# hungdinhxuan/real-time-deepfake-speech-detection

Hardware: AMD Instinct MI355X
Metric: utterances/sec (4 s @ 16 kHz) (higher is better)
Workload: dtype fp16

## Files before the change

### include/afx.h

```cpp
#ifndef AFX_H_
#define AFX_H_

#include <stddef.h>
#include <stdint.h>

#ifdef __cplusplus
extern "C" {
#endif

typedef struct afx_engine* afx_handle;

enum { AFX_ARCH_SSL = 0, AFX_ARCH_XLSR_AASIST = 1, AFX_ARCH_CONFORMER = 2,
       AFX_ARCH_CONFORMER_HEAD = 3  };
enum { AFX_EXTRACTOR_LAYER_NORM = 0,
       AFX_EXTRACTOR_GROUP_NORM = 1   };
enum { AFX_DT_BF16 = 0, AFX_DT_FP16 = 1, AFX_DT_FP32 = 2,
       AFX_DT_FP16X3 = 3  };

typedef struct afx_config {
  int arch;
  int dtype;
  int n_layers;
  int conf_emb;
  int conf_heads;
  int conf_kernel;
  int conf_blocks;
  int pre_emphasis;
  float pre_emphasis_coef;
  int extractor_mode;
} afx_config;

int afx_create(const afx_config* cfg, afx_handle* out);
void afx_destroy(afx_handle h);
const char* afx_last_error(void);
const char* afx_version(void);
const char* afx_build_id(void);
int afx_hip_versions(int* build, int* runtime);

int afx_load_weight(afx_handle h, const char* name, const float* dev_ptr, const int64_t* shape, int ndim,
                    void* stream);
int afx_finalize(afx_handle h, void* stream);

int afx_num_frames(int n_samples);
size_t afx_workspace_bytes(afx_handle h, int B, int L);
int afx_forward(afx_handle h, const float* wave, int B, int L, float* logits, void* ws, size_t ws_bytes,
                void* stream);
int afx_trunk_forward(afx_handle h, const float* wave, int B, int L, void* ws, size_t ws_bytes, void* stream);
int afx_head_from_workspace(afx_handle h, int B, int L, float* logits, void* ws, size_t ws_bytes, void* stream);
int afx_ssl_forward(afx_handle h, const float* wave, int B, int L, float* feats, void* ws, size_t ws_bytes,
                    void* stream);
size_t afx_ragged_workspace_bytes(afx_handle h, int B, int Lmax);
int afx_forward_ragged(afx_handle h, const float* wave, int B, int Lmax, const int* n_samples, float* logits, void* ws,
                       size_t ws_bytes, void* stream);
int afx_ssl_forward_ragged(afx_handle h, const float* wave, int B, int Lmax, const int* n_samples, float* feats,
                           int* n_frames, void* ws, size_t ws_bytes, void* stream);
size_t afx_tail_workspace_bytes(afx_handle h, int B, int T5);
int afx_tail_forward(afx_handle h, const void* conv5_h, int B, int T5, float* logits, void* ws, size_t ws_bytes,
                     void* stream);
int afx_tail_forward_strided(afx_handle h, const void* conv5_h, long batch_stride, int B, int T5, float* logits, void* ws,
                             size_t ws_bytes, void* stream);
size_t afx_tail_windows_workspace_bytes(afx_handle h, int B, int T5);
int afx_tail_forward_windows(afx_handle h, const void* conv5_h, long long total_elems, const long long* offs, int B, int T5,
                             float* logits, void* ws, size_t ws_bytes, void* stream);
typedef struct afx_kv afx_kv;
int afx_kv_create(afx_handle h, int n_streams, afx_kv** out);
void afx_kv_destroy(afx_kv* kv);
size_t afx_kv_state_bytes(const afx_kv* kv);
size_t afx_kv_workspace_bytes(const afx_kv* kv, int n_frames);
int afx_kv_step(afx_kv* kv, const float* feats6, int n_frames, float* logits, void* ws, size_t ws_bytes, void* stream);
int afx_kv_reset(afx_kv* kv, const int* slots, int n_slots, void* stream);
size_t afx_kv_ragged_workspace_bytes(const afx_kv* kv, int n_max);
int afx_kv_step_ragged(afx_kv* kv, const float* feats6, int n_max, const int* n_frames, float* logits, void* ws, size_t ws_bytes,
                       void* stream);
size_t afx_kv_active_workspace_bytes(const afx_kv* kv, int n_active, int n_max);
int afx_kv_step_active(afx_kv* kv, const int* slots, int n_active, const float* feats6, int n_max, const int* n_frames,
                       float* logits, void* ws, size_t ws_bytes, void* stream);
#define AFX_KV_META 8
size_t afx_kv_slot_bytes(const afx_kv* kv);
int afx_kv_export(afx_kv* kv, const int* slots, int n, void* payload, int* meta, void* stream);
int afx_kv_import(afx_kv* kv, const int* slots, int n, const void* payload, const int* meta, void* stream);
int afx_head_forward(afx_handle h, const float* feats, int B, int T, float* logits, void* ws, size_t ws_bytes,
                     void* stream);
size_t afx_head_workspace_bytes(afx_handle h, int B, int T);
int afx_conformer_forward(afx_handle h, const float* tokens, int B, int T, float* logits, float* embedding, void* ws,
                          size_t ws_bytes, void* stream);
int afx_check_finite(afx_handle h, void* stream);
int afx_enable_taps(afx_handle h, int on);
int afx_tap(afx_handle h, const char* name, float* out, size_t cap_elems, size_t* n_out, void* stream);

int afx_profile_begin(afx_handle h);
int afx_profile_end(afx_handle h, int n_classes, double* ms, double* flops, long long* launches);
int afx_profile_num_classes(void);
const char* afx_profile_class_name(int cls);

int afx_engine_set(afx_handle h, const char* key, int value);
int afx_engine_get(afx_handle h, const char* key, int* value);
int afx_gemm_plan(int M, int N, int K, int rpb, int kchunk, int groups, int flags, int objective, int* out);
int afx_conf_chain_waves(int M, int objective);
int afx_debug_set(const char* key, int value);

int afx_k_gemm(int dtype, const void* A, long lda, const void* W, long ldw, int M, int N, int K, const float* bias,
               int act, float alpha, const float* resid, long ldr, float* out_f, long ldo_f, void* out_h, long ldo_h,
               void* stream);
int afx_k_conv_gemm(int dtype, const void* in_h, const void* Wp, int B, int Tin, int Tout, int Cin, int k, int s,
                    int N, const float* bias, float* out_f, void* stream);
int afx_k_conv_ln_act(int dtype, const void* in_h, const void* Wp, int B, int Tin, int Tout, int Cin, int k, int s,
                      const float* bias, const float* gamma, const float* beta, float eps, int act, float* out_f,
                      void* out_h, void* stream);
int afx_k_pack_linear(int dtype, const float* w, int N, int K, int Kpad, void* out_h, void* stream);
int afx_k_pack_conv(int dtype, const float* w, int N, int Cin, int k, void* out_h, void* stream);
int afx_k_conv0(int dtype, const float* wave, int B, int L, const float* w, const float* bias, const float* gamma,
                const float* beta, int pre_emph, float coef, void* out_h, void* stream);
size_t afx_k_conv0_pack_bytes(void);
int afx_k_conv0_pack(const float* w, const float* bias, void* pack, void* stream);
int afx_k_conv0_packed(int dtype, const float* wave, int B, int L, const void* pack, const float* w, const float* bias,
                       const float* gamma, const float* beta, int pre_emph, float coef, void* out_h, void* stream);
int afx_k_pre_emphasis(const float* x, int B, int L, float coef, float* y, void* stream);
int afx_k_tile_crop(const float* x, const long long* offs, const long long* starts, int B, int duration, float* out,
                    void* stream);
int afx_k_resample(const float* x, const long long* in_offs, const long long* out_offs, int B, long long max_out,
                   const float* taps, int L, int M, int T, float* out, void* stream);
int afx_k_resample_stream(const float* x, int A, int n_in, float* hist, const int* slot, const float* taps, int L, int M,
                          int T, float* out, void* stream);
int afx_k_ingest(const void* stage, long long stage_bytes, const int* hdr, int rows, int max_out, int encoding,
                 const float* taps, int L, int M, int T, float* hist, float* ring, int S, int ring_len, void* stream);
typedef struct afx_ingest_format {
  const float* taps;
  int encoding, L, M, T;
} afx_ingest_format;
int afx_k_ingest_mixed(const void* stage, long long stage_bytes, const int* hdr, int rows, const afx_ingest_format* formats,
                       int n_formats, const int* max_out, float* hist, int Hs, float* ring, int S, int ring_len, void* stream);
int afx_k_ingest_pop(const float* ring, int S, int ring_len, const int* table, int A, int hop, float* out, void* stream);
int afx_k_payload_expand(void* stage, long long stage_bytes, const int* hdr, int rows, int max_n, void* stream);
int afx_k_jitter_place(const void* stage, long long stage_bytes, const int* hdr, int rows, int max_n, int encoding,
                       float* jring, int S, int J, void* stream);
int afx_k_jitter_place_mixed(const void* stage, long long stage_bytes, const int* hdr, int rows, int max_n, float* jring, int S,
                             int J, void* stream);
int afx_k_jitter_conceal(float* jring, int S, int J, const int* hdr, int rows, int max_n, const float* fade, int P, int F,
                         int mode, void* stream);
int afx_k_jitter_release(const float* jring, int S, int J, const int* hdr, int rows, int max_out, const float* taps, int L,
                         int M, int T, float* ring, int ring_len, void* stream);
typedef struct afx_jitter_rate {
  const float* taps;
  const float* fade;
  int L, M, T, J, P, F;
} afx_jitter_rate;
int afx_k_jitter_place_rates(const void* stage, long long stage_bytes, const int* hdr, int rows, int max_n,
                             const afx_jitter_rate* rates, int n_rates, float* jring, int S, int Js, void* stream);
int afx_k_jitter_conceal_rates(float* jring, int S, int Js, const int* hdr, int rows, int max_n, const afx_jitter_rate* rates,
                               int n_rates, int mode, void* stream);
int afx_k_jitter_release_rates(const float* jring, int S, int Js, const int* hdr, int rows, const afx_jitter_rate* rates,
                               int n_rates, const int* max_out, float* ring, int ring_len, void* stream);
int afx_k_jitter_noise(float* jring, int S, int J, const int* hdr, int rows, int max_n, unsigned seed, const float* amp,
                       void* stream);
int afx_k_jitter_noise_rates(float* jring, int S, int Js, const int* hdr, int rows, int max_n, const afx_jitter_rate* rates,
                             int n_rates, unsigned seed, const float* amp, void* stream);
typedef struct afx_jitter_lags {
  int Pmin, Pmax, Wc, P0, Hd;
} afx_jitter_lags;
int afx_k_jitter_pitch(const float* jring, int S, int J, const int* hdr, int rows, int Pmin, int Pmax, int Wc, int P0, int* period,
                       void* stream);
int afx_k_jitter_pitch_rates(const float* jring, int S, int Js, const int* hdr, int rows, const afx_jitter_rate* rates,
                             const afx_jitter_lags* lags, int n_rates, int* period, void* stream);
int afx_k_jitter_conceal_period(float* jring, int S, int J, const int* hdr, int rows, int max_n, const float* gain,
                                const int* period, int Pmin, int Pmax, int P0, int Hd, int F, void* stream);
int afx_k_jitter_conceal_period_rates(float* jring, int S, int Js, const int* hdr, int rows, int max_n, const afx_jitter_rate* rates,
                                      const afx_jitter_lags* lags, int n_rates, const int* period, void* stream);
int afx_k_gate(const float* x, int A, int n, const int* hdr, int frame, float e_floor, float ratio, float rise, int hang,
               float* nf, int* h, float* ring, int S, int ring_len, int* kept, unsigned char* mask, void* stream);
int afx_k_gate_la(const float* x, int A, int n, const int* hdr, int frame, float e_floor, float ratio, float rise, int hang,
                  int pre, float* nf, int* h, int* flags, float* line, float* ring, int* src, int S, int ring_len, int* kept,
                  unsigned char* mask, void* stream);
int afx_k_gate_tone(const float* x, int A, int n, const int* hdr, int frame, float e_floor, float ratio, float rise, int hang,
                    const float* coef, int K, float thr, int confirm, int hold, float* nf, int* h, int* tone_state, float* ring,
                    int S, int ring_len, int* kept, int* ntone, unsigned char* mask, float* tsum, void* stream);
int afx_k_turn(const float* staging, int S, int ring_len, const unsigned char* mask, const int* hdr, int A, int F, int frame,
               int min_frames, int max_frames, float* bufs, int* state, int* totals, int* done, void* stream);
int afx_k_turn_collect(const float* bufs, int S, int max_frames, int frame, const int* rows, int R, float* out, void* stream);
int afx_k_turn_close(const int* slots, int A, int S, int min_frames, int max_frames, int* state, int* totals, int* done,
                     void* stream);
int afx_k_turn_scan(const unsigned char* mask, const long long* offs, int A, int min_frames, int max_frames, int close_end,
                    int* table, int cap, int* row_base, int* totals, int* open, void* stream);
int afx_k_turn_clips(const float* x, const long long* xoffs, int A, int frame, int max_frames, const int* table, int r0, int R,
                     float* out, void* stream);
int afx_k_cascade_store(const float* x, int A, int hop, const int* hdr, float* hist, int S, int window, void* stream);
int afx_k_cascade_select(const float* scores, int stride, const int* hdr, int A, int* wait, int* counts, int S,
                         float threshold, int budget, int cooldown, int* sel, void* stream);
int afx_k_cascade_windows(const float* hist, int S, int window, const int* hdr, int A, const int* sel, int budget,
// ... 42 lines not shown
```

### real-time-deepfake-speech-detection_amd/afx/_lib.py

```python
import ctypes as C
import os

_HERE = os.path.dirname(os.path.abspath(__file__))
LIB_PATH = os.environ.get("AFX_LIB") or os.path.join(os.path.dirname(_HERE), "lib", "libafx.so")

ARCH_SSL, ARCH_XLSR_AASIST, ARCH_CONFORMER, ARCH_CONFORMER_HEAD = 0, 1, 2, 3
DT_BF16, DT_FP16, DT_FP32, DT_FP16X3 = 0, 1, 2, 3
ACT_NONE, ACT_GELU, ACT_SWISH, ACT_SELU = 0, 1, 2, 3
KV_META = 8


class AfxError(RuntimeError):
    pass


class Config(C.Structure):
    _fields_ = [("arch", C.c_int), ("dtype", C.c_int), ("n_layers", C.c_int),
                ("conf_emb", C.c_int), ("conf_heads", C.c_int), ("conf_kernel", C.c_int),
                ("conf_blocks", C.c_int), ("pre_emphasis", C.c_int), ("pre_emphasis_coef", C.c_float),
                ("extractor_mode", C.c_int)]


_P, _I, _L, _F, _Z = C.c_void_p, C.c_int, C.c_long, C.c_float, C.c_size_t


class IngestFormat(C.Structure):
    _fields_ = [("taps", C.c_void_p), ("encoding", C.c_int), ("L", C.c_int), ("M", C.c_int), ("T", C.c_int)]


class JitterRate(C.Structure):
    _fields_ = [("taps", C.c_void_p), ("fade", C.c_void_p), ("L", C.c_int), ("M", C.c_int), ("T", C.c_int), ("J", C.c_int),
                ("P", C.c_int), ("F", C.c_int)]


class JitterLags(C.Structure):
    _fields_ = [("Pmin", C.c_int), ("Pmax", C.c_int), ("Wc", C.c_int), ("P0", C.c_int), ("Hd", C.c_int)]


SIGNATURES = {
    "afx_create": (_I, [C.POINTER(Config), C.POINTER(_P)]),
    "afx_destroy": (None, [_P]),
    "afx_last_error": (C.c_char_p, []),
    "afx_version": (C.c_char_p, []),
    "afx_build_id": (C.c_char_p, []),
    "afx_hip_versions": (_I, [C.POINTER(C.c_int), C.POINTER(C.c_int)]),
    "afx_load_weight": (_I, [_P, C.c_char_p, _P, C.POINTER(C.c_int64), _I, _P]),
    "afx_finalize": (_I, [_P, _P]),
    "afx_num_frames": (_I, [_I]),
    "afx_workspace_bytes": (_Z, [_P, _I, _I]),
    "afx_head_workspace_bytes": (_Z, [_P, _I, _I]),
    "afx_forward": (_I, [_P, _P, _I, _I, _P, _P, _Z, _P]),
    "afx_ssl_forward": (_I, [_P, _P, _I, _I, _P, _P, _Z, _P]),
    "afx_trunk_forward": (_I, [_P, _P, _I, _I, _P, _Z, _P]),
    "afx_head_from_workspace": (_I, [_P, _I, _I, _P, _P, _Z, _P]),
    "afx_head_forward": (_I, [_P, _P, _I, _I, _P, _P, _Z, _P]),
    "afx_ragged_workspace_bytes": (_Z, [_P, _I, _I]),
    "afx_forward_ragged": (_I, [_P, _P, _I, _I, C.POINTER(C.c_int), _P, _P, _Z, _P]),
    "afx_ssl_forward_ragged": (_I, [_P, _P, _I, _I, C.POINTER(C.c_int), _P, C.POINTER(C.c_int), _P, _Z, _P]),
    "afx_tail_workspace_bytes": (_Z, [_P, _I, _I]),
    "afx_tail_forward": (_I, [_P, _P, _I, _I, _P, _P, _Z, _P]),
    "afx_tail_forward_strided": (_I, [_P, _P, _L, _I, _I, _P, _P, _Z, _P]),
    "afx_tail_windows_workspace_bytes": (_Z, [_P, _I, _I]),
    "afx_tail_forward_windows": (_I, [_P, _P, C.c_longlong, C.POINTER(C.c_longlong), _I, _I, _P, _P, _Z, _P]),
    "afx_conformer_forward": (_I, [_P, _P, _I, _I, _P, _P, _P, _Z, _P]),
    "afx_engine_set": (_I, [_P, C.c_char_p, _I]),
    "afx_engine_get": (_I, [_P, C.c_char_p, C.POINTER(C.c_int)]),
    "afx_gemm_plan": (_I, [_I, _I, _I, _I, _I, _I, _I, _I, C.POINTER(C.c_int)]),
    "afx_conf_chain_waves": (_I, [_I, _I]),
    "afx_kv_create": (_I, [_P, _I, C.POINTER(_P)]),
    "afx_kv_destroy": (None, [_P]),
    "afx_kv_state_bytes": (_Z, [_P]),
    "afx_kv_workspace_bytes": (_Z, [_P, _I]),
    "afx_kv_step": (_I, [_P, _P, _I, _P, _P, _Z, _P]),
    "afx_kv_reset": (_I, [_P, _P, _I, _P]),
    "afx_kv_ragged_workspace_bytes": (_Z, [_P, _I]),
    "afx_kv_step_ragged": (_I, [_P, _P, _I, _P, _P, _P, _Z, _P]),
    "afx_kv_active_workspace_bytes": (_Z, [_P, _I, _I]),
    "afx_kv_step_active": (_I, [_P, _P, _I, _P, _I, _P, _P, _P, _Z, _P]),
    "afx_kv_slot_bytes": (_Z, [_P]),
    "afx_kv_export": (_I, [_P, _P, _I, _P, _P, _P]),
    "afx_kv_import": (_I, [_P, _P, _I, _P, _P, _P]),
    "afx_check_finite": (_I, [_P, _P]),
    "afx_enable_taps": (_I, [_P, _I]),
    "afx_tap": (_I, [_P, C.c_char_p, _P, _Z, C.POINTER(_Z), _P]),
    "afx_profile_begin": (_I, [_P]),
    "afx_profile_end": (_I, [_P, _I, C.POINTER(C.c_double), C.POINTER(C.c_double), C.POINTER(C.c_longlong)]),
    "afx_profile_num_classes": (_I, []),
    "afx_profile_class_name": (C.c_char_p, [_I]),
    "afx_debug_set": (_I, [C.c_char_p, _I]),
    "afx_k_gemm": (_I, [_I, _P, _L, _P, _L, _I, _I, _I, _P, _I, _F, _P, _L, _P, _L, _P, _L, _P]),
    "afx_k_conv_gemm": (_I, [_I, _P, _P, _I, _I, _I, _I, _I, _I, _I, _P, _P, _P]),
    "afx_k_conv_ln_act": (_I, [_I, _P, _P, _I, _I, _I, _I, _I, _I, _P, _P, _P, _F, _I, _P, _P, _P]),
    "afx_k_pack_linear": (_I, [_I, _P, _I, _I, _I, _P, _P]),
    "afx_k_pack_conv": (_I, [_I, _P, _I, _I, _I, _P, _P]),
    "afx_k_conv0": (_I, [_I, _P, _I, _I, _P, _P, _P, _P, _I, _F, _P, _P]),
    "afx_k_conv0_pack_bytes": (_Z, []),
    "afx_k_conv0_pack": (_I, [_P, _P, _P, _P]),
    "afx_k_conv0_packed": (_I, [_I, _P, _I, _I, _P, _P, _P, _P, _P, _I, _F, _P, _P]),
    "afx_k_pre_emphasis": (_I, [_P, _I, _I, _F, _P, _P]),
    "afx_k_tile_crop": (_I, [_P, _P, _P, _I, _I, _P, _P]),
    "afx_k_resample": (_I, [_P, _P, _P, _I, C.c_longlong, _P, _I, _I, _I, _P, _P]),
    "afx_k_resample_stream": (_I, [_P, _I, _I, _P, _P, _P, _I, _I, _I, _P, _P]),
    "afx_k_ingest": (_I, [_P, C.c_longlong, _P, _I, _I, _I, _P, _I, _I, _I, _P, _P, _I, _I, _P]),
    "afx_k_ingest_mixed": (_I, [_P, C.c_longlong, _P, _I, _P, _I, _P, _P, _I, _P, _I, _I, _P]),
    "afx_k_ingest_pop": (_I, [_P, _I, _I, _P, _I, _I, _P, _P]),
    "afx_k_payload_expand": (_I, [_P, C.c_longlong, _P, _I, _I, _P]),
    "afx_k_jitter_place": (_I, [_P, C.c_longlong, _P, _I, _I, _I, _P, _I, _I, _P]),
    "afx_k_jitter_place_mixed": (_I, [_P, C.c_longlong, _P, _I, _I, _P, _I, _I, _P]),
    "afx_k_jitter_conceal": (_I, [_P, _I, _I, _P, _I, _I, _P, _I, _I, _I, _P]),
    "afx_k_jitter_release": (_I, [_P, _I, _I, _P, _I, _I, _P, _I, _I, _I, _P, _I, _P]),
    "afx_k_jitter_place_rates": (_I, [_P, C.c_longlong, _P, _I, _I, _P, _I, _P, _I, _I, _P]),
    "afx_k_jitter_conceal_rates": (_I, [_P, _I, _I, _P, _I, _I, _P, _I, _I, _P]),
    "afx_k_jitter_release_rates": (_I, [_P, _I, _I, _P, _I, _P, _I, _P, _P, _I, _P]),
    "afx_k_jitter_noise": (_I, [_P, _I, _I, _P, _I, _I, C.c_uint, _P, _P]),
    "afx_k_jitter_noise_rates": (_I, [_P, _I, _I, _P, _I, _I, _P, _I, C.c_uint, _P, _P]),
    "afx_k_jitter_pitch": (_I, [_P, _I, _I, _P, _I, _I, _I, _I, _I, _P, _P]),
    "afx_k_jitter_pitch_rates": (_I, [_P, _I, _I, _P, _I, _P, _P, _I, _P, _P]),
    "afx_k_jitter_conceal_period": (_I, [_P, _I, _I, _P, _I, _I, _P, _P, _I, _I, _I, _I, _I, _P]),
    "afx_k_jitter_conceal_period_rates": (_I, [_P, _I, _I, _P, _I, _I, _P, _P, _I, _P, _P]),
    "afx_k_gate": (_I, [_P, _I, _I, _P, _I, _F, _F, _F, _I, _P, _P, _P, _I, _I, _P, _P, _P]),
    "afx_k_gate_la": (_I, [_P, _I, _I, _P, _I, _F, _F, _F, _I, _I, _P, _P, _P, _P, _P, _P, _I, _I, _P, _P, _P]),
    "afx_k_gate_tone": (_I, [_P, _I, _I, _P, _I, _F, _F, _F, _I, _P, _I, _F, _I, _I, _P, _P, _P, _P, _I, _I, _P, _P, _P, _P, _P]),
    "afx_k_turn": (_I, [_P, _I, _I, _P, _P, _I, _I, _I, _I, _I, _P, _P, _P, _P, _P]),
    "afx_k_turn_collect": (_I, [_P, _I, _I, _I, _P, _I, _P, _P]),
    "afx_k_turn_close": (_I, [_P, _I, _I, _I, _I, _P, _P, _P, _P]),
    "afx_k_turn_scan": (_I, [_P, _P, _I, _I, _I, _I, _P, _I, _P, _P, _P, _P]),
    "afx_k_turn_clips": (_I, [_P, _P, _I, _I, _I, _P, _I, _I, _P, _P]),
    "afx_k_cascade_store":(_I, [_P, _I, _I, _P, _P, _I, _I, _P]),
    "afx_k_cascade_select": (_I, [_P, _I, _P, _I, _P, _P, _I, _F, _I, _I, _P, _P]),
    "afx_k_cascade_windows": (_I, [_P, _I, _I, _P, _I, _P, _I, _P, _P]),
    "afx_k_verdict": (_I, [_P, _I, _P, _P, _I, _P, _P, _I, _F, _F, _F, _F, _I, _I, _I, _I, _P, _I, _P]),
    "afx_k_evidence_mark": (_I, [_P, _I, _P, _I, _I, _I, _P, _P, _P, _P, _I, _P, _P, _P]),
    "afx_k_evidence_copy": (_I, [_P, _P, _I, _P, _P, _I, _I, _I, _I, _P, _P, _I, _P, _P, _I, _I, _P]),
    "afx_k_quality": (_I, [_P, C.c_longlong, _I, _I, _P, _P, _I, _F, _I, _I, _F, _F, _I, _I, _I, _P, _I, _P, _P, _I, _P, _P, _P]),
    "afx_k_rownorm": (_I, [_I, _P, _L, _I, _I, _P, _P, _F, _I, _P, _L, _P, _L, _P]),
    "afx_k_mhsa": (_I, [_I, _P, _P, _I, _I, _I, _P]),
    "afx_k_conf_attn": (_I, [_I, _P, _L, _P, _L, _P, _I, _I, _I, _I, _I, _P, _L, _P]),
    "afx_k_conf_attn_mfma": (_I, [_I, _P, _L, _P, _L, _P, _I, _I, _I, _I, _I, _P, _L, _P]),
    "afx_k_conf_dwconv": (_I, [_I, _P, _L, _P, _P, _P, _P, _I, _I, _I, _I, _P, _L, _P]),
    "afx_aasist_error": (C.c_char_p, []),
    "afx_k_gat": (_I, [_P, _I, _I, _I, _I, _P, _P, _P, _P, _P, _P, _P, _P, _P, _F, _P, _P]),
    "afx_k_hgat": (_I, [_P, _I, _P, _I, _I, _I, _I, C.POINTER(_P), _F, _P, _L, _P, _P, _P, _P, _P]),
    "afx_k_resblock_scratch_floats": (_Z, [_I, _I, _I, _I, _I]),
    "afx_k_resblock": (_I, [_P, _I, _I, _I, _I, _I, _P, _P, _P, _P, _P, _P, _P, _P, _P, _P, _P]),
    "afx_k_graph_pool": (_I, [_P, _I, _I, _I, _I, _P, _P, _P, _P]),
}

_lib = None


def lib():
    global _lib
    if _lib is None:
        if not os.path.exists(LIB_PATH):
            raise AfxError(f"{LIB_PATH} is missing: the HIP library has not been built "
                           "(run __graft_entry__.build()); there is no CPU fallback")
        import torch
        l = C.CDLL(LIB_PATH)
        for name, (res, args) in SIGNATURES.items():
            fn = getattr(l, name)
            fn.restype, fn.argtypes = res, args
        _check_runtime(l)
        _lib = l
    return _lib


def _check_runtime(l):
    b, r = C.c_int(0), C.c_int(0)
    if l.afx_hip_versions(C.byref(b), C.byref(r)) != 0:
        raise AfxError(l.afx_last_error().decode())
    bm, rm = b.value // 10_000_000, r.value // 10_000_000
    if bm != rm:
        raise AfxError(f"libafx.so was built with HIP {bm}.x (HIP_VERSION {b.value}) but this process runs HIP runtime {rm}.x "
# ... 27 lines not shown
```

### real-time-deepfake-speech-detection_amd/afx/kernels.py

```python
import torch

from ._lib import ACT_GELU, ACT_NONE, ACT_SELU, ACT_SWISH, call_on, check, lib, ptr, stream_ptr
from .engine import DTYPES, torch_dtype

ACTS = {None: ACT_NONE, "gelu": ACT_GELU, "swish": ACT_SWISH, "selu": ACT_SELU}


def _out(out, shape, dtype, device):
    if out is None or out is False:
        return None
    if out is True:
        return torch.empty(*shape, dtype=dtype, device=device)
    assert out.dtype == dtype and tuple(out.shape) == tuple(shape) and out.stride(-1) == 1, (out.dtype, out.shape, out.stride())
    return out


def gemm(dtype, A, W, bias=None, act=None, alpha=1.0, resid=None, out_f=True, out_h=False):
    M, K = A.shape
    N = W.shape[0]
    of = _out(out_f, (M, N), torch.float32, A.device)
    oh = _out(out_h, (M, N), torch_dtype(dtype), A.device)
    check(call_on(A, lib().afx_k_gemm, DTYPES[dtype], ptr(A), A.stride(0), ptr(W), W.stride(0), M, N, K, ptr(bias), ACTS[act],
                           alpha, ptr(resid), N if resid is None else resid.stride(0), ptr(of), N if of is None else of.stride(0),
                           ptr(oh), N if oh is None else oh.stride(0)))
    return of, oh


def pack_linear(dtype, w, kpad=None):
    N, K = w.shape
    kpad = kpad or K
    out = torch.empty(N, kpad, dtype=torch_dtype(dtype), device=w.device)
    check(call_on(w, lib().afx_k_pack_linear, DTYPES[dtype], ptr(w), N, K, kpad, ptr(out)))
    return out


def pack_conv(dtype, w):
    N, Cin, k = w.shape
    out = torch.empty(N, k * Cin, dtype=torch_dtype(dtype), device=w.device)
    check(call_on(w, lib().afx_k_pack_conv, DTYPES[dtype], ptr(w), N, Cin, k, ptr(out)))
    return out


def _packed(out, shape, dtype, device):
    out = _out(out, shape, dtype, device)
    assert out is None or out.is_contiguous()
    return out


def conv_gemm(dtype, x_h, wp, k, s, bias=None, out=True):
    B, Tin, Cin = x_h.shape
    N = wp.shape[0]
    Tout = (Tin - k) // s + 1
    out = _packed(out, (B, Tout, N), torch.float32, x_h.device)
    check(call_on(x_h, lib().afx_k_conv_gemm, DTYPES[dtype], ptr(x_h), ptr(wp), B, Tin, Tout, Cin, k, s, N, ptr(bias), ptr(out)))
    return out


def conv_ln_act(dtype, x_h, wp, k, s, bias, gamma, beta, act="gelu", eps=1e-5, out_f=False, out_h=True):
    B, Tin, Cin = x_h.shape
    Tout = (Tin - k) // s + 1
    of = _packed(out_f, (B, Tout, 512), torch.float32, x_h.device)
    oh = _packed(out_h, (B, Tout, 512), torch_dtype(dtype), x_h.device)
    check(call_on(x_h, lib().afx_k_conv_ln_act, DTYPES[dtype], ptr(x_h), ptr(wp), B, Tin, Tout, Cin, k, s, ptr(bias), ptr(gamma),
                                  ptr(beta), eps, ACTS[act], ptr(of), ptr(oh)))
    return of, oh


def conv0(dtype, wave, w, bias, gamma, beta, pre_emph=False, coef=0.97):
    B, L = wave.shape
    T0 = (L - 10) // 5 + 1
    out = torch.empty(B, T0, 512, dtype=torch_dtype(dtype), device=wave.device)
    check(call_on(wave, lib().afx_k_conv0, DTYPES[dtype], ptr(wave), B, L, ptr(w), ptr(bias), ptr(gamma), ptr(beta),
                            1 if pre_emph else 0, coef, ptr(out)))
    return out


def conv0_pack(w, bias):
    pack = torch.empty(lib().afx_k_conv0_pack_bytes(), dtype=torch.uint8, device=w.device)
    check(call_on(w, lib().afx_k_conv0_pack, ptr(w), ptr(bias), ptr(pack)))
    return pack


def conv0_packed(dtype, wave, pack, w, bias, gamma, beta, pre_emph=False, coef=0.97):
    B, L = wave.shape
    T0 = (L - 10) // 5 + 1
    out = torch.empty(B, T0, 512, dtype=torch_dtype(dtype), device=wave.device)
    check(call_on(wave, lib().afx_k_conv0_packed, DTYPES[dtype], ptr(wave), B, L, ptr(pack), ptr(w), ptr(bias), ptr(gamma),
                  ptr(beta), 1 if pre_emph else 0, coef, ptr(out)))
    return out


def rownorm(dtype, x, gamma, beta, eps=1e-5, act=None, out_f=True, out_h=False):
    rows, Cc = x.shape
    of = _out(out_f, (rows, Cc), torch.float32, x.device)
    oh = _out(out_h, (rows, Cc), torch_dtype(dtype), x.device)
    check(call_on(x, lib().afx_k_rownorm, DTYPES[dtype], ptr(x), x.stride(0), rows, Cc, ptr(gamma), ptr(beta), eps, ACTS[act],
                              ptr(of), Cc if of is None else of.stride(0), ptr(oh), Cc if oh is None else oh.stride(0)))
    return of, oh


def mhsa(dtype, qkv, B, T, H):
    out = torch.empty(B * T, H * 64, dtype=torch_dtype(dtype), device=qkv.device)
    check(call_on(qkv, lib().afx_k_mhsa, DTYPES[dtype], ptr(qkv), ptr(out), B, T, H))
    return out


def conf_attn(dtype, q, kv, rel, B, N, H, dh, max_pos=512):
    out = torch.empty(B * N, H * dh, dtype=torch_dtype(dtype), device=q.device)
# ... 82 lines not shown
```

### real-time-deepfake-speech-detection_amd/csrc/afx_engine.hip

```cpp
#include <hip/hip_runtime.h>

#include <algorithm>
#include <cmath>
#include <cstdarg>
#include <cstdio>
#include <cstring>
#include <string>
#include <unordered_map>
#include <unordered_set>
#include <vector>

#include "../../include/afx.h"
#include "afx_common.h"
#include "afx_kernels.h"
#include "afx_aasist.h"
#include "afx_entry.h"

using namespace afx;

static thread_local char g_err[512] = "";
int afx::fail(const char* fmt, ...) {
  va_list ap;
  va_start(ap, fmt);
  vsnprintf(g_err, sizeof g_err, fmt, ap);
// ... 578 lines not shown
      return fail("afx_finalize: missing weight 'ssl_model.model.encoder.pos_conv.0.weight_g/weight_v'");
    }
    if (h->s3) KOK(launch_split_weight_rows(h->posw, kD, (kD / kPosG) * kPosK, h->wscale(h->posw, kD, (size_t)(kD / kPosG) * kPosK), s));
  }
  if (h->cfg.arch == AFX_ARCH_CONFORMER || head_only) {
    for (int b = 0; b < h->nblk; ++b) {
      ConfBlock& K = h->blk[b];
      if (fold_bn(h, "conformer.encoder_blocks." + std::to_string(b) + ".conv.net.5.", h->C2, K.bn_scale, K.bn_shift, s)) return 1;
      KOK(launch_pack_linear(K.rel32, 1025, h->dh, 64, K.rel_h, h->dt, s));
      if (h->E == 144) {
        auto put = [&](int st, int off, const float* v, int n) -> int {
          HIP_OK(hipMemcpyAsync(K.chain_prm[st] + off, v, (size_t)n * 4, hipMemcpyDeviceToDevice, s));
          return 0;
        };
        for (int st = 0; st < 3; ++st) HIP_OK(hipMemsetAsync(K.chain_prm[st], 0, (kChainParamFloats + kChainScaleFloats) * 4, s));
        for (int st = 0; st < 3; st += 2) {
          const ConfFF& ff = K.ff[st / 2];
          if (put(st, CP_FF_G, ff.ln.g, 144) || put(st, CP_FF_B, ff.ln.b, 144) || put(st, CP_FF_B1, ff.b1, 576) || put(st, CP_FF_B2, ff.b2, 144))
            return 1;
        }
        if (put(0, CP_LN2_G, K.attn_ln.g, 144) || put(0, CP_LN2_B, K.attn_ln.b, 144) ||
            put(1, CP_LN2_G, K.conv_ln.g, 144) || put(1, CP_LN2_B, K.conv_ln.b, 144) ||
            put(1, CP_BA, K.bout, 144) || put(1, CP_BB, K.bpw1, 576) ||
            put(2, CP_LN2_G, K.post_ln.g, 144) || put(2, CP_LN2_B, K.post_ln.b, 144) ||
            put(2, CP_BA, K.bpw2, 144))
          return 1;
        if (h->s3) {
          auto sc = [&](int st, int off, const void* w, int rows, int kp) -> int {
            HIP_OK(hipMemcpyAsync(K.chain_prm[st] + kChainParamFloats + off, h->wscale(w, rows, kp), (size_t)rows * 4, hipMemcpyDeviceToDevice, s));
            return 0;
          };
          if (sc(0, CS_FF1, K.ff[0].w1, h->FF, h->Ep) || sc(0, CS_FF2, K.ff[0].w2, h->E, h->FFp) || sc(0, CS_A, K.wqkv, 3 * h->inner, h->Ep) ||
              sc(1, CS_A, K.wout, h->E, h->Ep) || sc(1, CS_B, K.pw1, 2 * h->C2, h->Ep) ||
              sc(2, CS_A, K.pw2, h->E, h->C2p) || sc(2, CS_FF1, K.ff[1].w1, h->FF, h->Ep) || sc(2, CS_FF2, K.ff[1].w2, h->E, h->FFp))
            return 1;
        }
      }
    }
    if (head_only) {
      if (int rc = s3_layernorm_scales(h, lns, s)) return rc;
      h->finalized = true;
      return 0;
    }
    float w, b, m, v;
    HIP_OK(hipStreamSynchronize(s));
    HIP_OK(hipMemcpy(&w, h->F("first_bn.weight"), 4, hipMemcpyDeviceToHost));
    HIP_OK(hipMemcpy(&b, h->F("first_bn.bias"), 4, hipMemcpyDeviceToHost));
    HIP_OK(hipMemcpy(&m, h->F("first_bn.running_mean"), 4, hipMemcpyDeviceToHost));
    HIP_OK(hipMemcpy(&v, h->F("first_bn.running_var"), 4, hipMemcpyDeviceToHost));
    h->conf_bn_scale = w / sqrtf(v + kBnEps);
    h->conf_bn_shift = b - m * h->conf_bn_scale;
  } else if (h->cfg.arch == AFX_ARCH_XLSR_AASIST) {
    h->aw.split = h->s3 || h->dt != AFX_DT_FP32;
    if (const char* m = aasist_finalize(
            h->aw, [&](const std::string& k) { return h->F(k); }, [&](size_t bytes) { return h->dalloc(bytes); }, s))
      return fail("afx_finalize: %s", m);
  }
  if (int rc = s3_layernorm_scales(h, lns, s)) return rc;
  h->finalized = true;
  return 0;
}

struct Carver {
  char* base;
  size_t off = 0, largest = 0;
  explicit Carver(void* b) : base((char*)b) {}
  void* take(size_t bytes) {
    if (bytes > largest) largest = bytes;
    off = (off + 255) & ~(size_t)255;
    void* p = base ? base + off : nullptr;
    off += bytes;
    return p;
  }
};

struct Ws {
  int T[7];
  void *bufA = nullptr, *bufB = nullptr, *feats_h = nullptr, *xpad = nullptr, *hbuf = nullptr, *qkv = nullptr, *att = nullptr, *ff = nullptr,
       *ssl_h = nullptr;
  float *tmp32 = nullptr, *x = nullptr, *ssl_f = nullptr;
  void* s3planes = nullptr;
  size_t s3bytes = 0;
  float* gn_stats = nullptr;
  int* lens = nullptr;
  float *bucket_f = nullptr, *bucket_logits = nullptr;
  float *ll32 = nullptr, *xc = nullptr, *qkv32 = nullptr, *glu32 = nullptr;
  void *hc = nullptr, *hid = nullptr, *ao = nullptr, *u = nullptr;
  AasistWs aa;
};

static size_t carve(const afx_engine* e, int B, int L, int Tfeat, void* base, Ws* w, int T5 = 0, bool ragged = false) {
  Carver c(base);
  const size_t hs = dtype_size(e->dt);
  int T = Tfeat;
  w->lens = nullptr;
  w->bucket_f = w->bucket_logits = nullptr;
  if (L > 0 || T5 > 0) {
    if (L > 0) {
      conv_lengths(L, w->T);
      const size_t n0 = (size_t)B * w->T[0] * kC, n1 = (size_t)B * w->T[1] * kC;
      w->bufA = c.take(n0 * hs);
      w->bufB = c.take(n1 * hs);
      w->tmp32 = (float*)c.take(n1 * 4);
      if (e->cfg.extractor_mode == AFX_EXTRACTOR_GROUP_NORM) w->gn_stats = (float*)c.take(conv0_groupnorm_stats_floats(B, w->T[0]) * 4);
    } else {
      for (int i = 0; i < 5; ++i) w->T[i] = 0;
      w->T[5] = T5;
      w->T[6] = T5 >= kConvK[6] ? (T5 - kConvK[6]) / kConvS[6] + 1 : 0;
      w->bufA = w->bufB = nullptr;
      w->tmp32 = (float*)c.take((size_t)B * (w->T[6] > 0 ? w->T[6] : 1) * kC * 4);
    }
    T = w->T[6];
    w->feats_h = c.take((size_t)B * T * kC * hs);
    w->x = (float*)c.take((size_t)B * T * kD * 4);
    w->xpad = c.take((size_t)B * (T + kPosK) * kD * hs);
    w->hbuf = c.take((size_t)B * T * kD * hs);
    w->qkv = c.take((size_t)B * T * 3 * kD * hs);
    w->att = c.take((size_t)B * T * kD * hs);
    w->ff = c.take((size_t)B * T * kF * hs);
  }
  w->ssl_f = (float*)c.take((size_t)B * T * kD * 4);
  w->ssl_h = c.take((size_t)B * T * kD * hs);
  if (ragged) {
    w->lens = (int*)c.take((size_t)B * 4);
    if (e->cfg.arch == AFX_ARCH_XLSR_AASIST) {
      w->bucket_f = (float*)c.take((size_t)B * T * kD * 4);
      w->bucket_logits = (float*)c.take((size_t)B * 2 * 4);
    }
  }
  if (e->cfg.arch == AFX_ARCH_CONFORMER || e->cfg.arch == AFX_ARCH_CONFORMER_HEAD) {
    const size_t M = (size_t)B * (T + 1);
    w->ll32 = (float*)c.take((size_t)B * T * e->E * 4);
    w->xc = (float*)c.take(M * e->E * 4);
    w->qkv32 = (float*)c.take(M * 3 * e->inner * 4);
    w->glu32 = (float*)c.take(M * 2 * e->C2 * 4);
    w->hc = c.take(M * e->Ep * hs);
    w->hid = c.take(M * e->FFp * hs);
    w->ao = c.take(M * e->Ep * hs);
    w->u = c.take(M * e->C2p * hs);
  } else if (e->cfg.arch == AFX_ARCH_XLSR_AASIST) {
    aasist_carve(B, T, [&](size_t bytes) { return c.take(bytes); }, &w->aa);
  }
  w->s3planes = nullptr;
  w->s3bytes = 0;
  if (e->s3) {
    size_t big = c.largest;
    if (T5 > 0 && (size_t)B * T5 * kC * 4 > big) big = (size_t)B * T5 * kC * 4;
    w->s3bytes = big + 4096;
    w->s3planes = c.take(w->s3bytes);
  }
  return c.off + 256;
}

extern "C" int afx_num_frames(int n) {
  int T[7];
  conv_lengths(n, T);
  return T[6];
}

extern "C" size_t afx_workspace_bytes(afx_handle h, int B, int L) {
  if (!h || B <= 0 || L <= 0) return 0;
  Ws w;
  return carve(h, B, L, 0, nullptr, &w);
}

__global__ void half_to_f32_kernel(const uint16_t* in, float* out, size_t n, int is_bf16) {
  for (size_t i = (size_t)blockIdx.x * blockDim.x + threadIdx.x; i < n; i += (size_t)gridDim.x * blockDim.x) {
    if (is_bf16) {
      out[i] = __uint_as_float((unsigned)in[i] << 16);
    } else {
      _Float16 hv;
      memcpy(&hv, &in[i], 2);
      out[i] = (float)hv;
    }
  }
}
__global__ void pairs_to_f32_kernel(const uint16_t* in, float* out, size_t n, long ld, float inv_scale) {
  for (size_t i = (size_t)blockIdx.x * blockDim.x + threadIdx.x; i < n; i += (size_t)gridDim.x * blockDim.x) {
    const size_t r = i / ld;
    const long k = (long)(i - r * ld);
    const uint16_t* row = in + r * 2 * ld;
    _Float16 hi, lo;
    memcpy(&hi, &row[s3_pair_index(k)], 2);
    memcpy(&lo, &row[s3_pair_index(k) + 32], 2);
    out[i] = ((float)hi + (float)lo) * inv_scale;
  }
}
extern "C" int afx_tap(afx_handle h, const char* name, float* out, size_t cap, size_t* n_out, void* stream) {
  if (!h || !name) return fail("afx_tap: null argument");
  auto it = h->taps.find(name);
  if (it == h->taps.end()) return fail("afx_tap: no tap named '%s' (enable taps and run a forward first)", name);
  if (n_out) *n_out = it->second.n;
  if (out) {
    if (cap < it->second.n) return fail("afx_tap: buffer too small (%zu < %zu)", cap, it->second.n);
    HIP_OK(hipMemcpyAsync(out, it->second.p, it->second.n * 4, hipMemcpyDeviceToDevice, (hipStream_t)stream));
  }
  return 0;
}

enum ProfClass { PC_GEMM128 = 0, PC_GEMM64, PC_GEMM64_DEEP, PC_GEMM256, PC_GEMM_ROWLN, PC_GEMM8_256, PC_GEMM8_ROWLN, PC_GEMM_F32, PC_CONV0, PC_POSCONV, PC_ROWNORM, PC_MHSA, PC_CONF_ATTN, PC_CONF_DWCONV, PC_CONF_CHAIN,
                 PC_MISC, PC_AASIST, PC_COUNT };
static const char* kProfNames[PC_COUNT] = {"gemm_kernel<128x128>", "gemm_kernel<128x64>", "gemm_deep_kernel<128x64>", "gemm_kernel<256x256>",
                                           "gemm_kernel<128x512,rowLN>", "gemm8_kernel<256x256>", "gemm8_kernel<128x512,rowLN>", "gemm_f32_kernel<128x128>", "conv0_kernel", "posconv_kernel", "rownorm_kernel", "mhsa_kernel", "conf_attn_kernel",
                                           "conf_dwconv_kernel", "conf_chain_kernel", "misc", "aasist_head"};
struct ProfRec { int cls; hipEvent_t a, b; double flops; };
struct Profiler {
  bool on = false;
  std::vector<ProfRec> recs;
  std::vector<hipEvent_t> pool;
  size_t used = 0;
  hipEvent_t ev() {
    if (used == pool.size()) {
      hipEvent_t e;
      if (hipEventCreate(&e) != hipSuccess) return nullptr;
      pool.push_back(e);
    }
    return pool[used++];
  }
};
static void prof_forget(afx_engine* e) {
  if (!e->prof) return;
  for (hipEvent_t ev : e->prof->pool) (void)hipEventDestroy(ev);
  delete e->prof;
  e->prof = nullptr;
}

constexpr int kS3Bufs = 10;
struct S3Reg { const void* p; float scale; };
struct Call {
  afx_engine* const e;
  const hipStream_t s;
  const int objective;
  Profiler* const prof;
  void* const s3planes;
  const size_t s3bytes;
  const void* s3ok[kS3Bufs] = {nullptr};
  S3Reg s3reg[kS3Bufs] = {};

  Call(afx_engine* e_, void* stream, void* planes = nullptr, size_t bytes = 0, std::initializer_list<const void*> ok = {})
      : e(e_), s((hipStream_t)stream), objective(e_->concurrent ? OBJ_CU_TIME : OBJ_MAKESPAN), prof(e_->prof), s3planes(planes), s3bytes(bytes) {
    e->last_objective = dispatch_objective(objective);
    int i = 0;
    for (const void* p : ok)
      if (p && i < kS3Bufs) s3ok[i++] = p;
  }
  Call(afx_engine* e_, void* stream, const Ws& w)
      : Call(e_, stream, w.s3planes, w.s3bytes, {w.bufA, w.bufB, w.feats_h, w.hbuf, w.att, w.ff, w.xpad, w.hc, w.ssl_h, w.hid}) {}
  Call(const Call&) = delete;

  bool s3_ok(const void* p) const {
    if (!p || !s3planes) return false;
    for (const void* q : s3ok) if (q == p) return true;
    return false;
  }
  void s3_set(const void* p, float scale) {
    for (S3Reg& r : s3reg) if (r.p == p) { r.scale = scale; if (scale == 0.f) r.p = nullptr; return; }
    if (scale == 0.f) return;
    for (S3Reg& r : s3reg) if (!r.p) { r = S3Reg{p, scale}; return; }
  }
  float s3_pairs_in(const void* p) const {
    for (const S3Reg& r : s3reg) if (r.p && r.p == p) return r.scale;
    return 0.f;
  }
  template <class F>
  const char* timed(int cls, double flops, F&& f) {
    if (!prof || !prof->on) return f();
    hipEvent_t a = prof->ev(), b = prof->ev();
    if (!a || !b) return "profiler: hipEventCreate failed";
    (void)hipEventRecord(a, s);
    const char* m = f();
    (void)hipEventRecord(b, s);
    prof->recs.push_back({cls, a, b, flops});
    return m;
  }
  const char* gemm(const GemmArgs& g_in, int dt, int groups, bool rows = false);
  const char* rownorm(const RowNormArgs& a_in, const LnW& ln, int dt);
};
const char* Call::gemm(const GemmArgs& g_in, int dt, int groups, bool rows) {
  GemmArgs g = g_in;
  g.no_deep = e->gemm_small_deep ? 0 : 1;
  g.objective = objective;
  const double fl = 2.0 * g.M * g.N * (g.k_algo ? g.k_algo : g.K) * groups;
  auto cls_of = [](int tile) -> int {
    static const int cls[9] = {PC_GEMM128, PC_GEMM64, PC_GEMM256, PC_GEMM_ROWLN, PC_GEMM256, PC_GEMM256, PC_GEMM_ROWLN, PC_GEMM8_256, PC_GEMM8_ROWLN};
    return tile == 92 ? PC_GEMM64_DEEP : (tile >= 0 && tile < 9 ? cls[tile] : PC_GEMM128);
  };
  if (dt == DT_FP32 && s3planes) {
    const bool groups32 = !(g.K % 32 || g.kchunk % 32 || g.a_row % 32 || g.a_batch % 32 || g.g_a % 32 || g.kchunk_stride % 32 || g.ldw % 32 || g.g_w % 32);
    if (!groups32 || ((size_t)g.A & 15)) {
      if (rows) return "split-precision product with a row table: the operands must be pair-form addressable";
      if (g.out_h) s3_set(g.out_h, 0.f);
      return launch_gemm(g, DT_FP32, groups, s);
    }
    GemmArgs q = g;
    float a_scale = s3_pairs_in(g.A);
    if (a_scale == 0.f) {
      const long last = g.M - 1;
      long span = (last / g.rpb) * g.a_batch + (last % g.rpb) * g.a_row + (long)(g.K / g.kchunk - 1) * g.kchunk_stride + g.kchunk +
                  (long)(groups - 1) * g.g_a;
      span = (span + 31) & ~31L;
      if ((size_t)span * 4 > s3bytes) return "split-precision product: the A operand exceeds the pair-form scratch";
      a_scale = kS3ScaleFree;
      if (const char* m = timed(PC_MISC, 0, [&] { return launch_split_pairs((const float*)g.A, span, s3planes, a_scale, s); })) return m;
      q.A = s3planes;
    }
    q.k1 = g.K;
    q.K = 2 * g.K;
    if (!q.k_algo) q.k_algo = g.K;
    q.kchunk = 2 * g.kchunk;
    q.kchunk_stride = 2 * g.kchunk_stride;
    q.a_row = 2 * g.a_row;
    q.a_batch = 2 * g.a_batch;
    q.g_a = 2 * g.g_a;
    q.ldw = 2 * g.ldw;
    q.g_w = 2 * g.g_w;
    q.pre_scale = (const float*)((const char*)g.W + (size_t)groups * g.N * g.ldw * 4);
    q.a_inv = 1.0f / a_scale;
    if (g.out_h) {
      const bool pairs_out = s3_ok(g.out_h) && (g.N & 7) == 0 && (g.g_n & 7) == 0 && (g.ldo_h & 31) == 0 && g.out_h != g.A;
      q.oh_pairs = pairs_out ? 1 : 0;
      q.oh_scale = g.ln_gamma ? kS3ScaleBounded : kS3ScaleFree;
      s3_set(g.out_h, pairs_out ? q.oh_scale : 0.f);
    }
    const int tile = gemm_tile_of(q, groups);
    return timed(cls_of(tile), fl, [&] { return rows ? launch_gemm_rows(q, DT_FP16X3, s) : launch_gemm(q, DT_FP16X3, groups, s); });
  }
  if (rows && (dt == DT_FP32 || groups != 1)) return "gemm with a row table: half- or split-precision operands, one group";
  return timed(dt == DT_FP32 ? PC_GEMM_F32 : cls_of(gemm_tile_of(g, groups)), fl,
               [&] { return rows ? launch_gemm_rows(g, dt, s) : launch_gemm(g, dt, groups, s); });
}
const char* Call::rownorm(const RowNormArgs& a_in, const LnW& ln, int dt) {
  RowNormArgs a = a_in;
  a.gamma = ln.g; a.beta = ln.b;
  if (a.out_h && s3planes) {
    const bool pairs_out = dt == DT_FP32 && s3_ok(a.out_h) && (a.ldo_h & 31) == 0 && a.out_h != (const void*)a.x;
    a.oh_pairs = pairs_out ? 1 : 0;
    a.oh_scale = ln.scale;
    s3_set(a.out_h, pairs_out ? a.oh_scale : 0.f);
  }
  return timed(PC_ROWNORM, 0, [&] { return launch_rownorm(a, dt, s); });
}

static int tap(Call& cx, const char* name, const void* src, size_t n, bool is_half, long ld = 0) {
  afx_engine* e = cx.e;
  if (!e->taps_on) return 0;
  TapRec& t = e->taps[name];
  if (t.cap < n) {
    if (t.p) (void)hipFree(t.p);
    HIP_OK(hipMalloc((void**)&t.p, n * 4));
    t.cap = n;
  }
  t.n = n;
  const float pair_scale = is_half && e->s3 ? cx.s3_pairs_in(src) : 0.f;
  if (pair_scale != 0.f) {
    if (ld <= 0 || ld % 32 || n % ld) return fail("tap '%s': pair-form rows need a row stride that is a multiple of 32", name);
    hipLaunchKernelGGL(pairs_to_f32_kernel, dim3(1024), dim3(256), 0, cx.s, (const uint16_t*)src, t.p, n, ld, 1.0f / pair_scale);
    HIP_OK(hipGetLastError());
  } else if (is_half && e->dt != AFX_DT_FP32) {
    hipLaunchKernelGGL(half_to_f32_kernel, dim3(1024), dim3(256), 0, cx.s, (const uint16_t*)src, t.p, n,
                       e->dt == AFX_DT_BF16 ? 1 : 0);
    HIP_OK(hipGetLastError());
  } else {
    HIP_OK(hipMemcpyAsync(t.p, src, n * 4, hipMemcpyDeviceToDevice, cx.s));
  }
  return 0;
}

extern "C" int afx_profile_begin(afx_handle h) {
  if (!h) return fail("afx_profile_begin: null handle");
  if (!h->prof) h->prof = new Profiler();
  Profiler& p = *h->prof;
  p.on = true;
  p.recs.clear();
  p.used = 0;
  return 0;
}
extern "C" int afx_profile_end(afx_handle h, int n, double* ms, double* flops, long long* launches) {
  if (!h || n < PC_COUNT || !ms || !flops || !launches) return fail("afx_profile_end: need %d slots", (int)PC_COUNT);
  if (!h->prof) return fail("afx_profile_end: afx_profile_begin was not called on this handle");
  Profiler& p = *h->prof;
  for (int i = 0; i < n; ++i) { ms[i] = 0; flops[i] = 0; launches[i] = 0; }
  for (const ProfRec& r : p.recs) {
    HIP_OK(hipEventSynchronize(r.b));
    float t = 0;
    HIP_OK(hipEventElapsedTime(&t, r.a, r.b));
    ms[r.cls] += t;
    flops[r.cls] += r.flops;
    launches[r.cls] += 1;
  }
  p.on = false;
  p.recs.clear();
  p.used = 0;
  return 0;
}
extern "C" int afx_profile_num_classes(void) { return PC_COUNT; }
extern "C" const char* afx_profile_class_name(int c) { return c >= 0 && c < PC_COUNT ? kProfNames[c] : ""; }

static GemmArgs plain_gemm(const void* A, long lda, const void* W, long ldw, int M, int N, int K) {
  GemmArgs g;
  memset(&g, 0, sizeof g);
  g.A = A; g.W = W; g.M = M; g.N = N; g.K = K;
  g.rpb = M; g.a_batch = 0; g.a_row = lda;
  g.kchunk = K; g.kchunk_stride = 0; g.ldw = ldw;
  g.alpha = 1.f; g.act = ACT_NONE;
  g.o_batch_rows = M; g.oh_batch_rows = M;
  return g;
}

static RowNormArgs plain_norm(const float* x, long ldx, int rows, int C) {
  RowNormArgs a;
  memset(&a, 0, sizeof a);
  a.x = x; a.ldx = ldx; a.rows = rows; a.C = C; a.eps = kLnEps; a.act = ACT_NONE;
// ... 31 lines not shown
  if (!l5)
    KOK(cx.timed(PC_CONV0, 2.0 * B * T[0] * kC * kConvK[0], [&] {
      if (gn)
        return launch_conv0_groupnorm(wave, B, L, T[0], c0.w0, c0.gn_g, c0.gn_b, kLnEps,
                                      w.gn_stats, w.bufA, dt, s);
      if (e->s3) {
        const float sc = cx.s3_ok(w.bufA) ? c0.ln.scale : 0.f;
        cx.s3_set(w.bufA, sc);
        return launch_conv0(wave, B, L, T[0], c0.w0, c0.bias, c0.ln.g, c0.ln.b, e->cfg.pre_emphasis, e->cfg.pre_emphasis_coef, w.bufA, DT_FP16X3, s, e->conv0pack, sc);
      }
      return launch_conv0(wave, B, L, T[0], c0.w0, c0.bias, c0.ln.g, c0.ln.b, e->cfg.pre_emphasis, e->cfg.pre_emphasis_coef, w.bufA, dt, s,
                          e->conv0pack);
    }));
  if (!l5) TAP("c0", w.bufA, (size_t)B * T[0] * kC, true, kC);
  void* in = l5 ? const_cast<void*>(l5) : w.bufA;
  void* out = w.bufB;
  for (int i = l5 ? 6 : 1; i < 7; ++i) {
    const int M = B * T[i], K = kConvK[i] * kC;
    GemmArgs g = plain_gemm(in, 0, e->convw[i], K, M, kC, K);
    g.rpb = T[i]; g.a_batch = (l5 && i == 6 && l5_batch) ? l5_batch : (long)T[i - 1] * kC; g.a_row = (long)kConvS[i] * kC;
    g.o_batch_rows = T[i]; g.oh_batch_rows = T[i];
    g.bias = e->conv[i].bias;
    g.act = ACT_GELU;
    if (gn) {
      if (i < 6) {
        g.out_h = out; g.ldo_h = kC;
      } else {
        g.out_f = w.tmp32; g.ldo_f = kC;
      }
      KOK(cx.gemm(g, dt, 1));
    } else if (e->fuse_conv_ln && dt != DT_FP32) {
      g.ln_gamma = e->conv[i].ln.g; g.ln_beta = e->conv[i].ln.b; g.ln_eps = kLnEps;
      if (i < 6) {
        g.out_h = out; g.ldo_h = kC;
      } else {
        g.out_f = w.tmp32; g.ldo_f = kC;
      }
      KOK(cx.gemm(g, dt, 1));
    } else {
      g.act = ACT_NONE;
      g.out_f = w.tmp32; g.ldo_f = kC;
      KOK(cx.gemm(g, dt, 1));
      RowNormArgs n = plain_norm(w.tmp32, kC, M, kC);
      n.act = ACT_GELU;
      if (i < 6) {
        n.out_h = out; n.ldo_h = kC;
      } else {
        n.out_f = w.tmp32; n.ldo_f = kC;
      }
      KOK(cx.rownorm(n, e->conv[i].ln, dt));
    }
    if (i < 6) TAP("c" + std::to_string(i), out, (size_t)M * kC, true, kC);
    void* t = in; in = out; out = t;
  }
  const int Tt = T[6], M = B * Tt;
  if (tap(cx, "conv", w.tmp32, (size_t)M * kC, false)) return 1;
  {
    RowNormArgs n = plain_norm(w.tmp32, kC, M, kC);
    n.out_h = w.feats_h; n.ldo_h = kC;
    KOK(cx.rownorm(n, e->feat_ln, dt));
  }
  TAP("feats", w.feats_h, (size_t)M * kC, true, kC);
  {
    GemmArgs g = plain_gemm(w.feats_h, kC, e->projw, kC, M, kD, kC);
    g.rpb = Tt; g.a_batch = (long)Tt * kC; g.a_row = kC;
    g.bias = e->proj_b;
    g.out_f = w.x; g.ldo_f = kD; g.o_batch_rows = Tt; g.o_row_off = 0;
    g.out_h = w.xpad; g.ldo_h = kD; g.oh_batch_rows = Tt + kPosK; g.oh_row_off = kPosPad;
    KOK(cx.gemm(g, dt, 1));
    KOK(cx.timed(PC_MISC, 0, [&] { return launch_zero_pad_rows(w.xpad, B, Tt, kD, kPosPad, kPosK - kPosPad, dt, s, w.lens); }));
  }
  TAP("xpad", w.xpad, (size_t)B * (Tt + kPosK) * kD, true, kD);
  if (tap(cx, "proj", w.x, (size_t)M * kD, false)) return 1;
  if (e->posconv_sliding && dt != DT_FP32 && Tt <= 224) {
    PosConvArgs pc;
    memset(&pc, 0, sizeof pc);
    pc.xpad = w.xpad; pc.xpad_batch = (long)(Tt + kPosK) * kD; pc.W = e->posw; pc.bias = e->pos_b;
    pc.x = w.x; pc.B = B; pc.T = Tt;
    KOK(cx.timed(PC_POSCONV, 2.0 * M * kD * (kD / kPosG) * kPosK, [&] { return launch_posconv(pc, dt, s); }));
  } else {
    KOK(posconv_product(cx, w.xpad, Tt + kPosK, B, Tt, w.x, dt));
  }
  if (tap(cx, "pos", w.x, (size_t)M * kD, false)) return 1;
  auto resid_product = [&](const void* A, long lda, const void* W, int K, const float* bias) -> const char* {
    GemmArgs o = plain_gemm(A, lda, W, K, M, kD, K);
    o.bias = bias; o.resid = w.x; o.ldr = kD; o.out_f = w.x; o.ldo_f = kD;
    return cx.gemm(o, dt, 1);
  };
  for (int l = 0; l < e->cfg.n_layers; ++l) {
    const TrunkLayer& L = e->layers[l];
    RowNormArgs n1 = plain_norm(w.x, kD, M, kD);
    n1.out_h = w.hbuf; n1.ldo_h = kD;
    KOK(cx.rownorm(n1, L.ln1, dt));
    auto lp = [l](const char* leaf) { return "l" + std::to_string(l) + "." + leaf; };
    TAP(lp("ln1"), w.hbuf, (size_t)M * kD, true, kD);
    GemmArgs q = plain_gemm(w.hbuf, kD, L.wqkv, kD, M, 3 * kD, kD);
    q.bias = L.bqkv;
    q.out_h = w.qkv; q.ldo_h = 3 * kD;
    KOK(cx.gemm(q, dt, 1));
    TAP(lp("qkv"), w.qkv, (size_t)M * 3 * kD, true, 3 * kD);
    KOK(cx.timed(PC_MHSA, 4.0 * B * kH * (double)Tt * Tt * 64, [&] {
      if (e->s3 && Tt <= 224) {
        const bool pairs = cx.s3_ok(w.att);
        cx.s3_set(w.att, pairs ? kS3ScaleFree : 0.f);
        return launch_mhsa_split((const float*)w.qkv, (float*)w.att, B, Tt, kH, s, w.lens, pairs, kS3ScaleFree);
      }
      if (e->s3) cx.s3_set(w.att, 0.f);
      return launch_mhsa(w.qkv, w.att, B, Tt, kH, dt, s, w.lens);
    }));
    TAP(lp("att"), w.att, (size_t)M * kD, true, kD);
    KOK(resid_product(w.att, kD, L.wo, kD, L.bo));
    TAP(lp("mid"), w.x, (size_t)M * kD, false, kD);
    RowNormArgs n2 = plain_norm(w.x, kD, M, kD);
    n2.out_h = w.hbuf; n2.ldo_h = kD;
    KOK(cx.rownorm(n2, L.ln2, dt));
    TAP(lp("ln2"), w.hbuf, (size_t)M * kD, true, kD);
    GemmArgs f1 = plain_gemm(w.hbuf, kD, L.w1, kD, M, kF, kD);
    f1.bias = L.b1; f1.act = ACT_GELU;
    f1.out_h = w.ff; f1.ldo_h = kF;
    KOK(cx.gemm(f1, dt, 1));
    TAP(lp("ff"), w.ff, (size_t)M * kF, true, kF);
    KOK(resid_product(w.ff, kF, L.w2, kF, L.b2));
    if (e->taps_on) {
      const std::string nm = "layer" + std::to_string(l);
      if (tap(cx, nm.c_str(), w.x, (size_t)M * kD, false)) return 1;
    }
  }
  RowNormArgs nf = plain_norm(w.x, kD, M, kD);
  nf.out_f = w.ssl_f; nf.ldo_f = kD;
  nf.out_h = w.ssl_h; nf.ldo_h = kD;
  nf.nonfinite = e->nonfinite;
  nf.nf_lens = w.lens; nf.nf_rpb = Tt;
  KOK(cx.rownorm(nf, e->enc_ln, dt));
  if (tap(cx, "ssl", w.ssl_f, (size_t)M * kD, false)) return 1;
  TAP("ssl.op", w.ssl_h, (size_t)M * kD, true, kD);
  return 0;
}

static int run_conformer(Call& cx, int B, int T, Ws& w, float* logits, const float* tokens = nullptr, float* embedding = nullptr) {
  afx_engine* e = cx.e;
  const hipStream_t s = cx.s;
  const int dt = e->dt, E = e->E, Ep = e->Ep, N = T + 1, M = B * N;
  if (tokens) {
    KOK(cx.timed(PC_MISC, 0, [&] { return launch_conf_tokens(tokens, e->class_token, 1.f, 0.f, B, T, E, w.xc, s, true); }));
  } else {
    GemmArgs ll = plain_gemm(w.ssl_h, kD, e->conf_ll, kD, B * T, E, kD);
    ll.bias = e->ll_b;
    ll.out_f = w.ll32; ll.ldo_f = E;
    KOK(cx.gemm(ll, dt, 1));
    KOK(cx.timed(PC_MISC, 0, [&] {
      return launch_conf_tokens(w.ll32, e->class_token, e->conf_bn_scale, e->conf_bn_shift, B, T, E, w.xc, s);
    }));
  }
  if (tap(cx, "tokens", w.xc, (size_t)M * E, false)) return 1;
  const size_t hs = dtype_size(dt);
  const bool fused = e->fuse_conformer && (dt != DT_FP32 || e->s3) && E == 144 && e->inner == E && e->FFp == 4 * E && e->C2 == 2 * E;
  const int chain_dt = e->s3 ? DT_FP16X3 : dt;
  HIP_OK(hipMemsetAsync(w.ao, 0, (size_t)M * Ep * hs, s));
  if (!fused) {
    HIP_OK(hipMemsetAsync(w.hc, 0, (size_t)M * Ep * hs, s));
    HIP_OK(hipMemsetAsync(w.u, 0, (size_t)M * e->C2p * hs, s));
    if (e->FFp != e->FF) HIP_OK(hipMemsetAsync(w.hid, 0, (size_t)M * e->FFp * hs, s));
  }
  for (int b = 0; fused && b < e->nblk; ++b) {
    const ConfBlock& K = e->blk[b];
    ConfChainArgs c;
    memset(&c, 0, sizeof c);
    c.M = M; c.E = E; c.Ep = Ep; c.FFp = e->FFp; c.objective = cx.objective;
    c.x_in = w.xc; c.x_out = w.xc;
    auto ff = [&](const ConfFF& f) { c.ff_w1 = f.w1; c.ff_w2 = f.w2; };
    const double ff_fl = 2.0 * M * E * e->FF * 2;
    ff(K.ff[0]);
    c.params = K.chain_prm[0];
    c.w_a = K.wqkv; c.ld_w_a = Ep;
    c.out2 = w.qkv32; c.ld_out2 = 3 * e->inner;
    KOK(cx.timed(PC_CONF_CHAIN, ff_fl + 2.0 * M * E * 3 * e->inner, [&] { return launch_conf_chain(c, 0, chain_dt, s); }));
    auto bp = [b](const std::string& leaf) { return "b" + std::to_string(b) + "." + leaf; };
    TAP(bp("xa"), w.xc, (size_t)M * E, false, E);
    TAP(bp("qkv"), w.qkv32, (size_t)M * 3 * e->inner, false, 3 * e->inner);
    KOK(cx.timed(PC_CONF_ATTN, 6.0 * B * e->heads * (double)N * N * e->dh, [&] {
      if (e->conf_attn_mfma && dt != DT_FP32 && e->dh == 36)
        return launch_conf_attn_mfma(w.qkv32, 3 * e->inner, w.qkv32 + e->inner, 3 * e->inner, K.rel_h, 512, B, N, e->heads,
                                     e->dh, w.ao, Ep, dt, s, w.lens, 1);
      if (e->conf_attn_mfma && e->s3 && e->dh == 36 && N <= 209)
        return launch_conf_attn_split(w.qkv32, 3 * e->inner, w.qkv32 + e->inner, 3 * e->inner, (const float*)K.rel_h, 512, B, N,
                                      e->heads, e->dh, (float*)w.ao, Ep, s, w.lens, 1);
      return launch_conf_attn(w.qkv32, 3 * e->inner, w.qkv32 + e->inner, 3 * e->inner,
                              K.rel32, 512, B, N, e->heads, e->dh, w.ao, Ep, dt, s, w.lens, 1);
    }));
    TAP(bp("ao"), w.ao, (size_t)M * Ep, true, Ep);
    c.in_h = w.ao; c.ld_in_h = Ep;
    c.params = K.chain_prm[1];
    c.w_a = K.wout;
    c.w_b = K.pw1;
    c.out2 = w.glu32; c.ld_out2 = 2 * e->C2;
    KOK(cx.timed(PC_CONF_CHAIN, 2.0 * M * E * (e->inner + 2 * e->C2), [&] { return launch_conf_chain(c, 1, chain_dt, s); }));
    TAP(bp("xb"), w.xc, (size_t)M * E, false, E);
    TAP(bp("glu"), w.glu32, (size_t)M * 2 * e->C2, false, 2 * e->C2);
    KOK(cx.timed(PC_CONF_DWCONV, 2.0 * B * N * e->C2 * e->ck, [&] {
      return launch_conf_dwconv(w.glu32, 2 * e->C2, K.dw_w, K.dw_b, K.bn_scale, K.bn_shift, B, N, e->C2, e->ck, w.u, e->C2p, dt, s, w.lens, 1);
    }));
    TAP(bp("u"), w.u, (size_t)M * e->C2p, true, e->C2p);
    c.in_h = w.u; c.ld_in_h = e->C2p;
    c.params = K.chain_prm[2];
    c.w_a = K.pw2; c.ld_w_a = e->C2p;
// ... 1029 lines not shown
__global__ void f32_to_half_kernel(const float* in, uint16_t* out, size_t n, int is_bf16) {
  for (size_t i = (size_t)blockIdx.x * blockDim.x + threadIdx.x; i < n; i += (size_t)gridDim.x * blockDim.x) {
    if (is_bf16) {
      __bf16 v = (__bf16)in[i];
      memcpy(&out[i], &v, 2);
    } else {
      _Float16 v = (_Float16)in[i];
      memcpy(&out[i], &v, 2);
    }
  }
}

extern "C" int afx_head_forward(afx_handle h, const float* feats, int B, int T, float* logits, void* ws,
                                size_t ws_bytes, void* stream) {
  if (check_call(h, feats, B, T, logits, ws)) return 1;
  if (h->cfg.arch == AFX_ARCH_SSL) return fail("afx_head_forward: this handle has no back-end");
  if (h->cfg.arch == AFX_ARCH_CONFORMER_HEAD) return fail("afx_head_forward: this handle holds Conformer blocks only; use afx_conformer_forward");
  Ws w;
  memset(&w, 0, sizeof w);
  if (carve_ws("afx_head_forward", h, B, 0, T, ws, ws_bytes, &w)) return 1;
  hipStream_t s = (hipStream_t)stream;
  const size_t n = (size_t)B * T * kD;
  HIP_OK(hipMemcpyAsync(w.ssl_f, feats, n * 4, hipMemcpyDeviceToDevice, s));
  if (h->dt == AFX_DT_FP32) {
    HIP_OK(hipMemcpyAsync(w.ssl_h, feats, n * 4, hipMemcpyDeviceToDevice, s));
  } else {
    hipLaunchKernelGGL(f32_to_half_kernel, dim3(1024), dim3(256), 0, s, feats, (uint16_t*)w.ssl_h, n,
                       h->dt == AFX_DT_BF16 ? 1 : 0);
    HIP_OK(hipGetLastError());
  }
  Call cx(h, stream, w);
  return run_head(cx, B, T, w, logits);
}

extern "C" int afx_conformer_forward(afx_handle h, const float* tokens, int B, int T, float* logits, float* embedding,
                                     void* ws, size_t ws_bytes, void* stream) {
  if (check_call(h, tokens, B, T, logits, ws)) return 1;
  if (h->cfg.arch != AFX_ARCH_CONFORMER && h->cfg.arch != AFX_ARCH_CONFORMER_HEAD)
    return fail("afx_conformer_forward: this handle holds no Conformer blocks");
  Ws w;
  memset(&w, 0, sizeof w);
  if (carve_ws("afx_conformer_forward", h, B, 0, T, ws, ws_bytes, &w)) return 1;
  Call cx(h, stream, w);
  return run_conformer(cx, B, T, w, logits, tokens, embedding);
}

extern "C" size_t afx_head_workspace_bytes(afx_handle h, int B, int T) {
  if (!h || B <= 0 || T <= 0) return 0;
  Ws w;
  memset(&w, 0, sizeof w);
  return carve(h, B, 0, T, nullptr, &w);
}

extern "C" int afx_k_gemm(int dtype, const void* A, long lda, const void* W, long ldw, int M, int N, int K,
                          const float* bias, int act, float alpha, const float* resid, long ldr, float* out_f,
                          long ldo_f, void* out_h, long ldo_h, void* stream) {
  GemmArgs g = plain_gemm(A, lda, W, ldw, M, N, K);
  g.bias = bias; g.act = act; g.alpha = alpha; g.resid = resid; g.ldr = ldr;
  g.out_f = out_f; g.ldo_f = ldo_f; g.out_h = out_h; g.ldo_h = ldo_h;
  if (dtype == DT_FP16X3) {
    hipStream_t s = (hipStream_t)stream;
    if (K % 32 || lda != K || ldw != K || ((size_t)A & 15)) return fail("afx_k_gemm(fp16x3): contiguous 16-byte aligned rows, K %% 32 == 0");
    void *wp = nullptr, *planes = nullptr;
    const long span = ((long)M * K + 31) & ~31L;
    if (hipMalloc(&wp, (size_t)N * K * 4 + (size_t)N * 4) != hipSuccess || hipMalloc(&planes, (size_t)span * 4) != hipSuccess) {
      (void)hipFree(wp);
      return fail("afx_k_gemm(fp16x3): device allocation failed");
    }
    float* sc = (float*)((char*)wp + (size_t)N * K * 4);
    const char* m = launch_pack_linear((const float*)W, N, K, K, wp, DT_FP32, s);
    if (!m) m = launch_split_weight_rows(wp, N, K, sc, s);
    if (!m) m = launch_split_pairs((const float*)A, span, planes, kS3ScaleFree, s);
    if (!m) {
      g.A = planes; g.W = wp; g.k1 = K; g.K = 2 * K; g.kchunk = 2 * K; g.a_row = 2L * K; g.ldw = 2L * K; g.pre_scale = sc; g.a_inv = 1.0f / kS3ScaleFree;
      m = launch_gemm(g, DT_FP16X3, 1, s);
    }
    (void)hipStreamSynchronize(s);
    (void)hipFree(wp);
    (void)hipFree(planes);
    return m ? fail("%s", m) : 0;
  }
  KRET(launch_gemm(g, dtype, 1, (hipStream_t)stream));
}
extern "C" int afx_k_conv_gemm(int dtype, const void* in_h, const void* Wp, int B, int Tin, int Tout, int Cin, int k,
                               int s_, int N, const float* bias, float* out_f, void* stream) {
  GemmArgs g = plain_gemm(in_h, 0, Wp, (long)k * Cin, B * Tout, N, k * Cin);
  g.rpb = Tout; g.a_batch = (long)Tin * Cin; g.a_row = (long)s_ * Cin;
  g.o_batch_rows = Tout; g.oh_batch_rows = Tout;
  g.bias = bias; g.out_f = out_f; g.ldo_f = N;
  KRET(launch_gemm(g, dtype, 1, (hipStream_t)stream));
}
extern "C" int afx_k_conv_ln_act(int dtype, const void* in_h, const void* Wp, int B, int Tin, int Tout, int Cin,
                                 int k, int s_, const float* bias, const float* gamma, const float* beta, float eps,
                                 int act, float* out_f, void* out_h, void* stream) {
  GemmArgs g = plain_gemm(in_h, 0, Wp, (long)k * Cin, B * Tout, 512, k * Cin);
  g.rpb = Tout; g.a_batch = (long)Tin * Cin; g.a_row = (long)s_ * Cin;
  g.o_batch_rows = Tout; g.oh_batch_rows = Tout;
  g.bias = bias; g.act = act; g.ln_gamma = gamma; g.ln_beta = beta; g.ln_eps = eps;
  g.out_f = out_f; g.ldo_f = 512; g.out_h = out_h; g.ldo_h = 512;
  KRET(launch_gemm(g, dtype, 1, (hipStream_t)stream));
}
extern "C" int afx_k_pack_linear(int dtype, const float* w, int N, int K, int Kpad, void* out_h, void* stream) {
  KRET(launch_pack_linear(w, N, K, Kpad, out_h, dtype, (hipStream_t)stream));
}
extern "C" int afx_k_pack_conv(int dtype, const float* w, int N, int Cin, int k, void* out_h, void* stream) {
  KRET(launch_pack_conv(w, N, Cin, k, out_h, dtype, (hipStream_t)stream));
}
extern "C" size_t afx_k_conv0_pack_bytes(void) { return conv0_pack_bytes(); }
extern "C" int afx_k_conv0_pack(const float* w, const float* bias, void* pack, void* stream) {
  if (!w || !bias || !pack) return fail("afx_k_conv0_pack: null argument");
  KRET(launch_conv0_pack(w, bias, pack, (hipStream_t)stream));
}
extern "C" int afx_k_conv0_packed(int dtype, const float* wave, int B, int L, const void* pack, const float* w,
                                  const float* bias, const float* gamma, const float* beta, int pre_emph, float coef,
                                  void* out_h, void* stream) {
  if (dtype != DT_FP32 && !pack) return fail("afx_k_conv0_packed: null pack");
  KRET(launch_conv0(wave, B, L, (L - 10) / 5 + 1, w, bias, gamma, beta, pre_emph, coef, out_h, dtype, (hipStream_t)stream,
                    dtype != DT_FP32 ? pack : nullptr));
}
extern "C" int afx_k_conv0(int dtype, const float* wave, int B, int L, const float* w, const float* bias,
                           const float* gamma, const float* beta, int pre_emph, float coef, void* out_h,
                           void* stream) {
  void* pack = nullptr;
  if (dtype != DT_FP32) {
    if (hipMalloc(&pack, conv0_pack_bytes()) != hipSuccess) return fail("afx_k_conv0: device allocation failed");
    if (const char* m = launch_conv0_pack(w, bias, pack, (hipStream_t)stream)) {
      (void)hipFree(pack);
      return fail("%s", m);
    }
  }
  const char* m = launch_conv0(wave, B, L, (L - 10) / 5 + 1, w, bias, gamma, beta, pre_emph, coef, out_h, dtype,
                               (hipStream_t)stream, pack);
  if (pack) {
    (void)hipStreamSynchronize((hipStream_t)stream);
    (void)hipFree(pack);
  }
  if (m) return fail("%s", m);
  return 0;
}
extern "C" int afx_debug_set(const char* key, int value) {
  if (!key) return fail("afx_debug_set: null key");
  if (!strcmp(key, "gemm_map")) {
    gemm_set_map_mode(value);
    return 0;
  }
  if (!strcmp(key, "aasist_stop")) {
    aasist_set_stop(value);
    return 0;
  }
  if (!strcmp(key, "aasist_conv_slots")) {
    aasist_set_conv_slots(value);
    return 0;
  }
  if (!strcmp(key, "gemm_tile")) {
    gemm_set_tile(value);
    return 0;
  }
  if (!strcmp(key, "gemm_small_deep")) {
    gemm_set_small_deep(value);
    return 0;
  }
  if (!strcmp(key, "gemm_s3_small")) {
    gemm_set_s3_small(value);
    return 0;
  }
  if (!strcmp(key, "gemm_split")) {
// ... 24 lines not shown
    conf_chain_set_waves(value);
    return 0;
  }
  if (!strcmp(key, "conf_attn_waves")) {
    conf_attn_mfma_set_waves(value);
    return 0;
  }
  if (!strcmp(key, "mhsa_vtr")) {
    mhsa_set_vtr(value);
    return 0;
  }
  if (!strcmp(key, "mhsa_zsplit")) {
    mhsa_set_zsplit(value);
    return 0;
  }
  if (!strcmp(key, "mhsa_waves")) {
    mhsa_set_waves(value);
    return 0;
  }
  if (!strcmp(key, "mhsa_force_long")) {
    mhsa_set_force_long(value);
    return 0;
  }
  if (!strcmp(key, "conf_attn_force_long")) {
    conf_attn_mfma_set_force_long(value);
    return 0;
  }
  if (!strcmp(key, "conf_attn_block")) {
    conf_attn_set_block(value);
    return 0;
  }
  if (!strcmp(key, "gemm_deep")) {
    gemm_set_deep(value);
    return 0;
  }
  if (!strcmp(key, "gemm_nodma")) {
    if (!gemm_set_nodma(value)) return fail("afx_debug_set: gemm_nodma exists only in the attribution build (make attr, AFX_LIB=.../libafx_attr.so)");
    return 0;
  }
  if (!strcmp(key, "gemm_a_nt")) {
    gemm_set_a_nt(value);
    return 0;
  }
  if (!strcmp(key, "conv0_mfma")) {
    conv0_set_mfma(value);
    return 0;
  }

  return fail("afx_debug_set: unknown key '%s'", key);
}
extern "C" int afx_engine_set(afx_handle h, const char* key, int value) {
  if (!h || !key) return fail("afx_engine_set: null argument");
  if (!strcmp(key, "posconv_sliding")) h->posconv_sliding = value != 0;
  else if (!strcmp(key, "conf_attn_mfma")) h->conf_attn_mfma = value != 0;
  else if (!strcmp(key, "fuse_conformer")) h->fuse_conformer = value != 0;
  else if (!strcmp(key, "fuse_conv_ln")) h->fuse_conv_ln = value != 0;
  else if (!strcmp(key, "gemm_small_deep")) h->gemm_small_deep = value != 0;
  else if (!strcmp(key, "concurrent")) h->concurrent = value != 0;
  else return fail("afx_engine_set: unknown key '%s'", key);
  return 0;
}
extern "C" int afx_engine_get(afx_handle h, const char* key, int* value) {
  if (!h || !key || !value) return fail("afx_engine_get: null argument");
  if (!strcmp(key, "concurrent")) *value = h->concurrent;
  else if (!strcmp(key, "objective")) *value = h->last_objective;
  else return fail("afx_engine_get: unknown key '%s'", key);
  return 0;
}
extern "C" int afx_gemm_plan(int M, int N, int K, int rpb, int kchunk, int groups, int flags, int objective, int* out) {
  if (!out || M <= 0 || N <= 0 || K <= 0 || groups <= 0) return fail("afx_gemm_plan: bad arguments");
  GemmArgs g = plain_gemm(nullptr, K, nullptr, K, M, N, K);
  if (rpb > 0) g.rpb = rpb;
  if (kchunk > 0) g.kchunk = kchunk;
  if (flags & 1) g.ln_gamma = g.ln_beta = g.bias = (const float*)out;
  if (flags & 2) { g.k1 = K; g.K = 2 * K; g.kchunk = 2 * g.kchunk; }
  if (flags & 4) g.act = ACT_SWISH;
  if (flags & 8) g.no_deep = 1;
  const int obj = objective < 0 ? dispatch_objective(OBJ_MAKESPAN) : (objective ? OBJ_CU_TIME : OBJ_MAKESPAN);
  const GemmPlan pl = gemm_plan(g, groups, obj);
  out[0] = pl.family; out[1] = pl.tile; out[2] = pl.rows; out[3] = (int)pl.tiles;
  out[4] = pl.split_rows; out[5] = pl.rem_tile; out[6] = (int)pl.rem_tiles; out[7] = obj;
  return 0;
}
extern "C" int afx_conf_chain_waves(int M, int objective) {
  return conf_chain_waves_of(M, objective < 0 ? dispatch_objective(OBJ_MAKESPAN) : (objective ? OBJ_CU_TIME : OBJ_MAKESPAN));
}
extern "C" int afx_k_pre_emphasis(const float* x, int B, int L, float coef, float* y, void* stream) {
  KRET(launch_pre_emphasis(x, B, L, coef, y, (hipStream_t)stream));
}
extern "C" int afx_k_tile_crop(const float* x, const long long* offs, const long long* starts, int B, int duration,
                               float* out, void* stream) {
  if (!x || !offs || !out) return fail("afx_k_tile_crop: null argument");
  KRET(launch_tile_crop(x, offs, starts, B, duration, out, (hipStream_t)stream));
}
extern "C" int afx_k_rownorm(int dtype, const float* x, long ldx, int rows, int C, const float* gamma,
                             const float* beta, float eps, int act, float* out_f, long ldo_f, void* out_h, long ldo_h,
                             void* stream) {
  RowNormArgs a = plain_norm(x, ldx, rows, C);
  a.gamma = gamma; a.beta = beta; a.eps = eps; a.act = act; a.out_f = out_f; a.ldo_f = ldo_f; a.out_h = out_h; a.ldo_h = ldo_h;
  KRET(launch_rownorm(a, dtype, (hipStream_t)stream));
}
extern "C" int afx_k_mhsa(int dtype, const void* qkv, void* out, int B, int T, int H, void* stream) {
  if (dtype == DT_FP16X3) KRET(launch_mhsa_split((const float*)qkv, (float*)out, B, T, H, (hipStream_t)stream));
  KRET(launch_mhsa(qkv, out, B, T, H, dtype, (hipStream_t)stream));
}
extern "C" int afx_k_conf_attn(int dtype, const float* q, long ldq, const float* kv, long ldkv, const float* rel,
                               int max_pos, int B, int N, int H, int dh, void* out_h, long ldo, void* stream) {
  KRET(launch_conf_attn(q, ldq, kv, ldkv, rel, max_pos, B, N, H, dh, out_h, ldo, dtype, (hipStream_t)stream));
}
extern "C" int afx_k_conf_attn_mfma(int dtype, const float* q, long ldq, const float* kv, long ldkv, const void* rel_h,
                                    int max_pos, int B, int N, int H, int dh, void* out_h, long ldo, void* stream) {
  if (dtype == DT_FP16X3)
    KRET(launch_conf_attn_split(q, ldq, kv, ldkv, (const float*)rel_h, max_pos, B, N, H, dh, (float*)out_h, ldo, (hipStream_t)stream));
  KRET(launch_conf_attn_mfma(q, ldq, kv, ldkv, rel_h, max_pos, B, N, H, dh, out_h, ldo, dtype, (hipStream_t)stream));
}
extern "C" int afx_k_conf_dwconv(int dtype, const float* x, long ldx, const float* w, const float* bias,
                                 const float* bn_scale, const float* bn_shift, int B, int N, int C, int k, void* out_h,
                                 long ldo, void* stream) {
  KRET(launch_conf_dwconv(x, ldx, w, bias, bn_scale, bn_shift, B, N, C, k, out_h, ldo, dtype, (hipStream_t)stream));
}
```

### real-time-deepfake-speech-detection_amd/csrc/afx_frontend.hip

```cpp
#include <type_traits>

#include "afx_common.h"
#include "afx_kernels.h"

namespace afx {

constexpr int C0_FB = 64;
static int g_conv0_mfma = 1;

template <class HT>
__global__ __launch_bounds__(256) void conv0_kernel(const float* __restrict__ wave, int L, int T0,
                                                    const float* __restrict__ w, const float* __restrict__ bias,
                                                    const float* __restrict__ gamma, const float* __restrict__ beta,
                                                    int pre_emph, float pre_coef, typename HT::T* __restrict__ out) {
  typedef typename HT::T T;
  typedef typename HT::V8 V8;
  __shared__ float xs[C0_FB * 5 + 8];
  const int b = blockIdx.y;
  const int f0 = blockIdx.x * C0_FB;
  const int tid = threadIdx.x, lane = tid & 63, wv = tid >> 6;
  const float* x = wave + (long)b * L;
  const int s0 = f0 * 5;
  for (int i = tid; i < C0_FB * 5 + 5; i += 256) {
    const int gidx = s0 + i;
    float v = 0.f;
    if (gidx < L) {
      v = x[gidx];
      if (pre_emph) {
        const int gp = gidx > 0 ? gidx - 1 : 1;
        v -= pre_coef * x[gp];
      }
    }
    xs[i] = v;
  }
  float wr[8][10], bi[8], ga[8], be[8];
#pragma unroll
  for (int i = 0; i < 8; ++i) {
    const int c = lane * 8 + i;
#pragma unroll
    for (int j = 0; j < 10; ++j) wr[i][j] = w[c * 10 + j];
    bi[i] = bias[c];
    ga[i] = gamma[c];
    be[i] = beta[c];
  }
  __syncthreads();
  const int fend = min(C0_FB, T0 - f0);
  for (int f = wv; f < fend; f += 4) {
    float xv[10];
#pragma unroll
    for (int j = 0; j < 10; ++j) xv[j] = xs[f * 5 + j];
    float v[8];
    float sum = 0.f;
#pragma unroll
    for (int i = 0; i < 8; ++i) {
      float a = bi[i];
#pragma unroll
      for (int j = 0; j < 10; ++j) {
        a = fmaf(wr[i][j], xv[j], a);
        scalar_only(a);
      }
      v[i] = a;
      sum += a;
    }
#ifdef AFX_C0_KEEPX
#pragma unroll
    for (int j = 0; j < 10; ++j) asm volatile("" ::"v"(xv[j]), "v"(sum));
#endif
    const float mean = wave_sum(sum) * (1.0f / 512.0f);
    float sq = 0.f;
#pragma unroll
    for (int i = 0; i < 8; ++i) {
      v[i] -= mean;
      sq = fmaf(v[i], v[i], sq);
    }
    const float rstd = 1.0f / sqrtf(wave_sum(sq) * (1.0f / 512.0f) + 1e-5f);
    V8 o;
#pragma unroll
    for (int i = 0; i < 8; i += 2) {
      const f32x2_t yin = f32x2_t{fmaf(v[i] * rstd, ga[i], be[i]), fmaf(v[i + 1] * rstd, ga[i + 1], be[i + 1])};
      const f32x2_t y = sizeof(T) == 4 ? gelu_erf2(yin) : gelu_poly2(yin);
      o[i] = (T)y[0];
      o[i + 1] = (T)y[1];
    }
    *(V8*)(out + ((long)b * T0 + f0 + f) * 512 + lane * 8) = o;
  }
}
// ... 409 lines not shown
  dim3 grid((T0 + C0_FB - 1) / C0_FB, B);
  AFX_DISPATCH_HT(dtype, hipLaunchKernelGGL(conv0_gn_apply_kernel<HT>, grid, dim3(256), 0, s, wave, L, T0, w, mean, rstd, gamma,
                                            beta, (HT::T*)out_h));
  hipError_t e = hipGetLastError();
  return e == hipSuccess ? nullptr : hipGetErrorString(e);
}
size_t conv0_groupnorm_stats_floats(int B, int T0) { return (size_t)B * (((size_t)T0 + GN_FB - 1) / GN_FB * 1024 + 1024); }

const char* launch_conv0(const float* wave, int B, int L, int T0, const float* w, const float* bias,
                         const float* gamma, const float* beta, int pre_emph, float pre_coef, void* out_h,
                         int dtype, hipStream_t s, const void* wpack, float pair_scale) {
  if (B <= 0 || L < 10 || T0 != (L - 10) / 5 + 1) return "conv0: bad shape";
  if (dtype == DT_FP16X3) {
    if (!wpack) return "conv0 (fp16x3): the packed operand block is missing";
    dim3 grid((T0 + C0M_FB - 1) / C0M_FB, B);
    hipLaunchKernelGGL(conv0_split_kernel<F32T>, grid, dim3(256), 0, s, wave, L, T0, (const _Float16*)wpack, gamma, beta, pre_emph,
                       pre_coef, (float*)out_h, pair_scale);
    hipError_t e = hipGetLastError();
    return e == hipSuccess ? nullptr : hipGetErrorString(e);
  }
  if (dtype != DT_FP32 && g_conv0_mfma == 1 && wpack) {
    dim3 grid((T0 + C0M_FB - 1) / C0M_FB, B);
    if (dtype == DT_BF16)
      hipLaunchKernelGGL(conv0_split_kernel<BF16>, grid, dim3(256), 0, s, wave, L, T0, (const _Float16*)wpack, gamma, beta,
                         pre_emph, pre_coef, (__bf16*)out_h, 0.f);
    else
      hipLaunchKernelGGL(conv0_split_kernel<FP16>, grid, dim3(256), 0, s, wave, L, T0, (const _Float16*)wpack, gamma, beta,
                         pre_emph, pre_coef, (_Float16*)out_h, 0.f);
    hipError_t e = hipGetLastError();
    return e == hipSuccess ? nullptr : hipGetErrorString(e);
  }
  if (dtype != DT_FP32 && g_conv0_mfma) {
    dim3 grid((T0 + C0M_FB - 1) / C0M_FB, B);
    if (dtype == DT_BF16)
      hipLaunchKernelGGL(conv0_mfma_kernel<BF16>, grid, dim3(256), 0, s, wave, L, T0, w, bias, gamma, beta, pre_emph,
                         pre_coef, (__bf16*)out_h);
    else
      hipLaunchKernelGGL(conv0_mfma_kernel<FP16>, grid, dim3(256), 0, s, wave, L, T0, w, bias, gamma, beta, pre_emph,
                         pre_coef, (_Float16*)out_h);
    hipError_t e = hipGetLastError();
    return e == hipSuccess ? nullptr : hipGetErrorString(e);
  }
  dim3 grid((T0 + C0_FB - 1) / C0_FB, B);
  AFX_DISPATCH_HT(dtype, hipLaunchKernelGGL(conv0_kernel<HT>, grid, dim3(256), 0, s, wave, L, T0, w, bias, gamma, beta,
                                            pre_emph, pre_coef, (HT::T*)out_h));
  hipError_t e = hipGetLastError();
  return e == hipSuccess ? nullptr : hipGetErrorString(e);
}
void conv0_set_mfma(int v) { g_conv0_mfma = v; }

__global__ void pre_emphasis_kernel(const float* __restrict__ x, int L, float coef, float* __restrict__ y) {
  const long base = (long)blockIdx.y * L;
  for (int i = blockIdx.x * blockDim.x + threadIdx.x; i < L; i += gridDim.x * blockDim.x) {
    const int p = i > 0 ? i - 1 : (L > 1 ? 1 : 0);
    y[base + i] = x[base + i] - coef * x[base + p];
  }
}
const char* launch_pre_emphasis(const float* x, int B, int L, float coef, float* y, hipStream_t s) {
  if (B <= 0 || L <= 0) return "pre_emphasis: empty input";
  hipLaunchKernelGGL(pre_emphasis_kernel, dim3(min((L + 255) / 256, 1024), B), dim3(256), 0, s, x, L, coef, y);
  hipError_t e = hipGetLastError();
  return e == hipSuccess ? nullptr : hipGetErrorString(e);
}

__global__ void tile_crop_kernel(const float* __restrict__ x, const long long* __restrict__ offs,
                                 const long long* __restrict__ starts, int duration, float* __restrict__ out) {
  const int b = blockIdx.y;
  const long long o = offs[b], n = offs[b + 1] - o;
  long long p = starts ? starts[b] : 0;
  for (int i = blockIdx.x * blockDim.x + threadIdx.x; i < duration; i += gridDim.x * blockDim.x)
    out[(long)b * duration + i] = x[o + (p + i) % n];
}
const char* launch_tile_crop(const float* x, const long long* offs, const long long* starts, int B, int duration,
                             float* out, hipStream_t s) {
  if (B <= 0 || duration <= 0) return "tile_crop: empty batch";
  hipLaunchKernelGGL(tile_crop_kernel, dim3(min((duration + 255) / 256, 256), B), dim3(256), 0, s, x, offs, starts,
                     duration, out);
  hipError_t e = hipGetLastError();
  return e == hipSuccess ? nullptr : hipGetErrorString(e);
}

template <class HT, int RPW>
__global__ __launch_bounds__(256) void rownorm_kernel(RowNormArgs a) {
  typedef typename HT::T T;
  typedef typename HT::V4 V4;
  const int lane = threadIdx.x & 63;
  const long r0 = ((long)blockIdx.x * 4 + (threadIdx.x >> 6)) * RPW;
  if (r0 >= a.rows) return;
  f32x4 v[RPW][4];
  bool live[RPW];
#pragma unroll
  for (int u = 0; u < RPW; ++u) {
    live[u] = r0 + u < a.rows;
    const float* x = a.x + (live[u] ? r0 + u : r0) * a.ldx;
#pragma unroll
    for (int it = 0; it < 4; ++it) {
      const int c = (it * 64 + lane) * 4;
      v[u][it] = f32x4{0.f, 0.f, 0.f, 0.f};
      if (c < a.C) v[u][it] = *(const f32x4*)(x + c);
    }
  }
  f32x4 gm[4], bt[4];
#pragma unroll
  for (int it = 0; it < 4; ++it) {
    const int c = (it * 64 + lane) * 4;
    gm[it] = bt[it] = f32x4{0.f, 0.f, 0.f, 0.f};
    if (c < a.C) {
      gm[it] = *(const f32x4*)(a.gamma + c);
      bt[it] = *(const f32x4*)(a.beta + c);
    }
  }
  const float inv = 1.0f / (float)a.C;
#pragma unroll
  for (int u = 0; u < RPW; ++u) {
    if (!live[u]) continue;
    const long r = r0 + u;
    float sum = 0.f;
#pragma unroll
    for (int it = 0; it < 4; ++it) sum += (v[u][it][0] + v[u][it][1]) + (v[u][it][2] + v[u][it][3]);
    const float mean = wave_sum(sum) * inv;
    float sq = 0.f;
#pragma unroll
    for (int it = 0; it < 4; ++it) {
      const int c = (it * 64 + lane) * 4;
      if (c < a.C) {
#pragma unroll
        for (int i = 0; i < 4; ++i) {
          v[u][it][i] -= mean;
          sq = fmaf(v[u][it][i], v[u][it][i], sq);
        }
      }
    }
    const float var = wave_sum(sq) * inv;
    const float rstd = 1.0f / sqrtf(var + a.eps);
    if (a.nonfinite && lane == 0 && !(fabsf(mean) <= 3.0e38f && var <= 3.0e38f) &&
        (!a.nf_lens || (int)(r % a.nf_rpb) < a.nf_lens[r / a.nf_rpb]))
      atomicAdd(a.nonfinite, 1);
    const long orow = (r / a.rpb) * a.o_batch_rows + (r % a.rpb) + a.o_row_off;
    auto emit = [&](auto with_act) {
#pragma unroll
      for (int it = 0; it < 4; ++it) {
        const int c = (it * 64 + lane) * 4;
        if (c < a.C) {
          const f32x4 g = gm[it], b = bt[it];
          f32x4 y;
#pragma unroll
          for (int i = 0; i < 4; ++i) {
            y[i] = fmaf(v[u][it][i] * rstd, g[i], b[i]);
            if (decltype(with_act)::value) y[i] = apply_act(y[i], a.act);
          }
          if (a.out_f) *(f32x4*)(a.out_f + orow * a.ldo_f + c) = y;
          if (a.out_h) {
            if (std::is_same<T, float>::value && a.oh_pairs) {
              f16x4 hi, lo;
#pragma unroll
              for (int i = 0; i < 4; ++i) {
                const float sv = y[i] * a.oh_scale;
                hi[i] = (_Float16)sv;
                lo[i] = (_Float16)(sv - (float)hi[i]);
              }
              _Float16* hp = (_Float16*)a.out_h + orow * (2 * a.ldo_h) + s3_pair_index(c);
              *(f16x4*)hp = hi;
              *(f16x4*)(hp + 32) = lo;
            } else {
              V4 h;
#pragma unroll
              for (int i = 0; i < 4; ++i) h[i] = (T)y[i];
              *(V4*)((T*)a.out_h + orow * a.ldo_h + c) = h;
            }
          }
        }
      }
    };
    if (a.act == ACT_NONE) emit(std::false_type{});
    else emit(std::true_type{});
  }
}

const char* launch_rownorm(const RowNormArgs& a, int dtype, hipStream_t s) {
  if (a.rows <= 0 || a.C <= 0 || a.C > 1024 || a.C % 4) return "rownorm: need 0 < C <= 1024, C % 4 == 0";
  if (!a.out_f && !a.out_h) return "rownorm: no output";
  if (((size_t)a.x & 15) || (a.ldx & 3) || ((size_t)a.gamma & 15) || ((size_t)a.beta & 15))
    return "rownorm: input rows must start on 16-byte boundaries (x, gamma, beta 16-byte aligned; ldx % 4 == 0)";
  if (a.out_f && (((size_t)a.out_f & 15) || (a.ldo_f & 3))) return "rownorm: fp32 output rows must start on 16-byte boundaries (out_f 16-byte aligned, ldo_f % 4 == 0)";
  if (a.out_h && (((size_t)a.out_h & (dtype == DT_FP32 || dtype == DT_FP16X3 ? 15 : 7)) || (a.ldo_h & 3)))
    return "rownorm: operand-type output rows must start on the store's boundary (halfs: out_h 8-byte aligned, fp32: 16-byte; ldo_h % 4 == 0)";
  if (a.rows >= 16384) {
    AFX_DISPATCH_HT(dtype, hipLaunchKernelGGL((rownorm_kernel<HT, 2>), dim3((a.rows + 7) / 8), dim3(256), 0, s, a));
  } else {
    AFX_DISPATCH_HT(dtype, hipLaunchKernelGGL((rownorm_kernel<HT, 1>), dim3((a.rows + 3) / 4), dim3(256), 0, s, a));
  }
  hipError_t e = hipGetLastError();
  return e == hipSuccess ? nullptr : hipGetErrorString(e);
}

__global__ void zero_pad_rows_kernel(uint16_t* buf, int T, int C, int pf, int pb, const int* __restrict__ lens) {
  const int b = blockIdx.y;
  const int keep = lens ? lens[b] : T;
  const int rows = pf + pb + (T - keep);
  const long per = (long)(pf + T + pb) * C;
  for (long i = (long)blockIdx.x * blockDim.x + threadIdx.x; i < (long)rows * C / 8; i += (long)gridDim.x * blockDim.x) {
    const long e = i * 8;
    int r = (int)(e / C);
    const int c = (int)(e % C);
    if (r >= pf) r += keep;
    *(u32x4*)(buf + b * per + (long)r * C + c) = u32x4{0u, 0u, 0u, 0u};
  }
}
const char* launch_zero_pad_rows(void* buf_h, int B, int T, int C, int pf, int pb, int dtype, hipStream_t s, const int* lens) {
  if (C % 8) return "zero_pad_rows: C % 8 != 0";
  if (dtype == DT_FP32) C *= 2;
  hipLaunchKernelGGL(zero_pad_rows_kernel, dim3(32, B), dim3(256), 0, s, (uint16_t*)buf_h, T, C, pf, pb, lens);
  hipError_t e = hipGetLastError();
  return e == hipSuccess ? nullptr : hipGetErrorString(e);
}

template <class HT>
__global__ void pack_linear_kernel(const float* w, int N, int K, int Kpad, typename HT::T* out) {
  const long total = (long)N * Kpad;
  for (long i = (long)blockIdx.x * blockDim.x + threadIdx.x; i < total; i += (long)gridDim.x * blockDim.x) {
    const int n = (int)(i / Kpad), k = (int)(i % Kpad);
    out[i] = (typename HT::T)(k < K ? w[(long)n * K + k] : 0.f);
  }
}
const char* launch_pack_linear(const float* w, int N, int K, int Kpad, void* out_h, int dtype, hipStream_t s) {
  const int blocks = (int)min((long)4096, ((long)N * Kpad + 255) / 256);
  AFX_DISPATCH_HT(dtype, hipLaunchKernelGGL(pack_linear_kernel<HT>, dim3(blocks), dim3(256), 0, s, w, N, K, Kpad,
                                            (HT::T*)out_h));
  hipError_t e = hipGetLastError();
  return e == hipSuccess ? nullptr : hipGetErrorString(e);
}

template <class HT>
__global__ void pack_conv_kernel(const float* w, int N, int Cin, int k, typename HT::T* out) {
  const long total = (long)N * Cin * k;
  for (long i = (long)blockIdx.x * blockDim.x + threadIdx.x; i < total; i += (long)gridDim.x * blockDim.x) {
    const int n = (int)(i / ((long)Cin * k));
    const int rem = (int)(i % ((long)Cin * k));
    const int j = rem / Cin, c = rem % Cin;
    out[i] = (typename HT::T)w[((long)n * Cin + c) * k + j];
  }
}
const char* launch_pack_conv(const float* w, int N, int Cin, int k, void* out_h, int dtype, hipStream_t s) {
  const int blocks = (int)min((long)4096, ((long)N * Cin * k + 255) / 256);
  AFX_DISPATCH_HT(dtype, hipLaunchKernelGGL(pack_conv_kernel<HT>, dim3(blocks), dim3(256), 0, s, w, N, Cin, k,
                                            (HT::T*)out_h));
  hipError_t e = hipGetLastError();
  return e == hipSuccess ? nullptr : hipGetErrorString(e);
}

__global__ void posconv_norm_kernel(const float* v, int C, int cpg, int k, float* norm) {
  const int j = blockIdx.x;
  float s = 0.f;
  for (long i = threadIdx.x; i < (long)C * cpg; i += blockDim.x) {
    const float x = v[i * k + j];
    s = fmaf(x, x, s);
  }
  __shared__ float red[4];
  s = wave_sum(s);
// ... 99 lines not shown
```

### real-time-deepfake-speech-detection_amd/csrc/afx_gemm.hip

```cpp
#include "afx_common.h"
#include "afx_kernels.h"

#include <type_traits>

#ifdef AFX_ATTR
#define AFX_DBG(p, bit) ((p).dbg_nodma & (bit))
#else
#define AFX_DBG(p, bit) 0
#endif

namespace afx {

__device__ __forceinline__ void store_pairs8(void* out_h, long hrow, long ldo_h, long col, const f32x4& va, const f32x4& vb, float scale) {
  f16x8 hi, lo;
#pragma unroll
  for (int r = 0; r < 4; ++r) {
    const float sa = va[r] * scale, sb = vb[r] * scale;
    hi[r] = (_Float16)sa;
    hi[4 + r] = (_Float16)sb;
    lo[r] = (_Float16)(sa - (float)hi[r]);
    lo[4 + r] = (_Float16)(sb - (float)hi[4 + r]);
  }
  _Float16* hp = (_Float16*)out_h + hrow * (2 * ldo_h) + s3_pair_index(col);
  *(f16x8*)hp = hi;
  *(f16x8*)(hp + 32) = lo;
}

template <class HT, int BM, int BN, int WR, int WC, bool ROWLN, bool LEAN = false, bool S3 = false, bool ROWTAB = false>
__device__ __forceinline__ void gemm_epilogue(const GemmArgs& p, f32x4 (&acc)[BM / WR / 16][BN / WC / 16], char* smem,
                                              int m0, int n0, int g) {
  typedef typename HT::T T;
  typedef typename HT::V8 V8;
  typedef typename HT::V4 V4;
  constexpr int WM = BM / WR, WN = BN / WC;
  constexpr int MT = WM / 16, NT = WN / 16;
  const int tid = threadIdx.x, lane = tid & 63;
  const int wave = __builtin_amdgcn_readfirstlane(tid >> 6);
  const int wr = wave / WC, wc = wave % WC;
  if constexpr (ROWLN) {
    static_assert(BN % (16 * WC) == 0, "row-complete tile");
    __syncthreads();
    float* red = (float*)smem;
    float* vec = red + WC * BM;
    for (int t = tid; t < BN; t += 64 * WR * WC) {
      vec[t] = p.bias[n0 + t];
      vec[BN + t] = p.ln_gamma[n0 + t];
      vec[2 * BN + t] = p.ln_beta[n0 + t];
      if constexpr (S3) vec[3 * BN + t] = p.pre_scale[n0 + t] * p.a_inv;
    }
    __syncthreads();
    const int kq = lane >> 4;
#pragma unroll
    for (int j = 0; j < NT; ++j) {
      const f32x4 b = *(const f32x4*)(vec + wc * WN + j * 16 + 4 * kq);
      if constexpr (S3) {
        const f32x4 rs = *(const f32x4*)(vec + 3 * BN + wc * WN + j * 16 + 4 * kq);
#pragma unroll
        for (int i = 0; i < MT; ++i) acc[i][j] = acc[i][j] * rs + b;
      } else {
#pragma unroll
        for (int i = 0; i < MT; ++i) acc[i][j] += b;
      }
    }
    float mean[MT], rstd[MT];
    const float invn = 1.0f / (float)BN;
#pragma unroll
    for (int i = 0; i < MT; ++i) {
      float s = 0.f;
#pragma unroll
      for (int j = 0; j < NT; ++j) s += (acc[i][j][0] + acc[i][j][1]) + (acc[i][j][2] + acc[i][j][3]);
      s = rows_sum(s);
      if (kq == 0) red[wc * BM + wr * WM + i * 16 + (lane & 15)] = s;
    }
    __syncthreads();
#pragma unroll
    for (int i = 0; i < MT; ++i) {
      const int row = wr * WM + i * 16 + (lane & 15);
      float s = 0.f;
#pragma unroll
      for (int c = 0; c < WC; ++c) s += red[c * BM + row];
      mean[i] = s * invn;
    }
    __syncthreads();
#pragma unroll
    for (int i = 0; i < MT; ++i) {
      float s = 0.f;
#pragma unroll
      for (int j = 0; j < NT; ++j)
#pragma unroll
        for (int r = 0; r < 4; ++r) {
          acc[i][j][r] -= mean[i];
// ... 363 lines not shown
  const int nk = p.K >> 6;

  const unsigned lds_base = (unsigned)(size_t)smem;
  auto dma16 = [&](const T* src, unsigned lds_off, bool nt) {
    unsigned keep;
    const unsigned dst = __builtin_amdgcn_readfirstlane(lds_base + lds_off);
    if (nt)
      asm volatile("s_mov_b32 %0, m0\n\ts_mov_b32 m0, %2\n\ts_nop 0\n\tglobal_load_lds_dwordx4 %1, off nt\n\ts_mov_b32 m0, %0"
                   : "=&s"(keep) : "v"(src), "s"(dst) : "memory");
    else
      asm volatile("s_mov_b32 %0, m0\n\ts_mov_b32 m0, %2\n\ts_nop 0\n\tglobal_load_lds_dwordx4 %1, off\n\ts_mov_b32 m0, %0"
                   : "=&s"(keep) : "v"(src), "s"(dst) : "memory");
  };
  auto stage = [&](int buf, int kt) {
    const int k0 = kt << 6;
    const long ka = (long)(k0 / p.kchunk) * p.kchunk_stride + (k0 % p.kchunk);
    const unsigned base = (unsigned)(buf * STAGE);
    if constexpr (ASM_DMA) {
#pragma unroll
      for (int i = 0; i < AI; ++i) dma16(a_src[i] + ka, base + (i * NW + wave) * 1024, p.a_nt != 0);
#pragma unroll
      for (int i = 0; i < WI; ++i) dma16(w_src[i] + k0, base + A_BYTES + (i * NW + wave) * 1024, false);
    } else {
#pragma unroll
      for (int i = 0; i < AI; ++i)
        __builtin_amdgcn_global_load_lds((const __attribute__((address_space(1))) void*)(a_src[i] + ka),
                                         (__attribute__((address_space(3))) void*)(smem + base + (i * NW + wave) * 1024),
                                         16, 0, 0);
#pragma unroll
      for (int i = 0; i < WI; ++i)
        __builtin_amdgcn_global_load_lds((const __attribute__((address_space(1))) void*)(w_src[i] + k0),
                                         (__attribute__((address_space(3))) void*)(smem + base + A_BYTES + (i * NW + wave) * 1024),
                                         16, 0, 0);
    }
  };

  const int frow = lane & 15;
  const int fsw = (frow >> 1) & 7;
  const int a_off = (wr * WM + frow) * 128;
  const int w_off = A_BYTES + (wc * WN + frow) * 128;

  stage(0, 0);
  for (int kt = 0; kt < nk; ++kt) {
    asm volatile("s_waitcnt vmcnt(0)" ::: "memory");
    __syncthreads();
    if (kt + 1 < nk) stage((kt + 1) & 1, kt + 1);
    const char* sb = smem + (kt & 1) * STAGE;
    if constexpr (S3) {
      V8 af[2][MT], wf[2][NT];
#pragma unroll
      for (int ks = 0; ks < 2; ++ks) {
        const int slot = ((ks * 4 + (lane >> 4)) ^ fsw) * 16;
#pragma unroll
        for (int j = 0; j < NT; ++j) wf[ks][j] = *(const V8*)(sb + w_off + j * 16 * 128 + slot);
#pragma unroll
        for (int i = 0; i < MT; ++i) af[ks][i] = *(const V8*)(sb + a_off + i * 16 * 128 + slot);
      }
      __builtin_amdgcn_s_setprio(1);
      s3_mfma<HT, MT, NT>(wf[0], wf[1], af[0], af[1], acc);
      __builtin_amdgcn_s_setprio(0);
    } else {
#pragma unroll
      for (int ks = 0; ks < 2; ++ks) {
        const int slot = ((ks * 4 + (lane >> 4)) ^ fsw) * 16;
        V8 af[MT], wf[NT];
#pragma unroll
        for (int j = 0; j < NT; ++j) wf[j] = *(const V8*)(sb + w_off + j * 16 * 128 + slot);
#pragma unroll
        for (int i = 0; i < MT; ++i) af[i] = *(const V8*)(sb + a_off + i * 16 * 128 + slot);
        __builtin_amdgcn_s_setprio(1);
#pragma unroll
        for (int i = 0; i < MT; ++i)
#pragma unroll
          for (int j = 0; j < NT; ++j) acc[i][j] = HT::mfma(wf[j], af[i], acc[i][j]);
        __builtin_amdgcn_s_setprio(0);
      }
    }
  }

  gemm_epilogue<HT, BM, BN, WR, WC, ROWLN, LEAN, S3, ROWTAB>(p, acc, smem, m0, n0, g);
}


template <class HT, int BM, int BN, bool ROWLN, int MF = BM / 32, int PH = 1, bool TS = false, bool S3 = false, bool ROWTAB = false>
__global__ __launch_bounds__(512) void gemm8_kernel(GemmArgs p) {
  static_assert(!ROWTAB || !ROWLN, "per-batch output rows: wide-store epilogue only");
  typedef typename HT::T T;
  typedef typename HT::V8 V8;
  constexpr bool WIDE = BN > BM;
  constexpr int RA = BM / 2, RB = BN / 2;
  constexpr int FR = 16, KSN = 2;
  constexpr int MTH = RA / 2 / FR, NTH = RB / 4 / FR;
  constexpr int DA = RA / 64, DB = RB / 64;
  constexpr int OFF_A0 = 0, OFF_A1 = RA * 128, OFF_B0 = 2 * RA * 128, OFF_B1 = OFF_B0 + RB * 128;
  constexpr int BUF = 2 * (RA + RB) * 128;
  static_assert((WIDE ? MTH : NTH) * KSN == 4 && (WIDE ? NTH : MTH) * KSN == 8, "resident operand: 4 reads per half, flowing: 8");
  static_assert(2 * (WIDE ? DA : DB) + (WIDE ? DB : DA) == 6, "vmcnt(6) leaves R0, F0, R1 of tile t+2 in flight");
  static_assert(MF == BM / 32 || (!WIDE && MF >= 5 && MF < 8) || (WIDE && MF >= 2 && MF < 4), "short tiles: 160..224 of 256 rows, 64 / 96 of 128");
  constexpr int MF0 = (MF + 1) / 2, MF1 = MF - MF0;
  constexpr int BMC = (MF0 + MF1) * 32;
  extern __shared__ __attribute__((aligned(16))) char smem[];

  const int tid = threadIdx.x, lane = tid & 63;
  const int wave = __builtin_amdgcn_readfirstlane(tid >> 6);
  const int wr = wave >> 2, wc = wave & 3;
  const int g = blockIdx.z;
  const T* Ag = (const T*)p.A + (long)g * p.g_a;
  const T* Wg = (const T*)p.W + (long)g * p.g_w;
  const int nN = (p.N + BN - 1) / BN, nM = (p.M - p.m_lo + BMC - 1) / BMC;
  const int nwg = nM * nN;
  const int nk = p.K >> 6;

  const T* srcA[2][DA];
  const T* srcB[2][DB];
  int m0 = 0, n0 = 0;
  auto setup = [&](int v) {
    int pm, pn;
    int L = v;
    if (p.map_mode >= 1) {
      const int q = nwg >> 3, r = nwg & 7, xcd = L & 7;
      L = (xcd < r ? xcd * (q + 1) : r * (q + 1) + (xcd - r) * q) + (L >> 3);
    }
    if (p.map_mode == 2) {
      constexpr int GM = 8;
      const int width = GM * nN, grp = L / width, first = grp * GM;
      const int gsz = nM - first < GM ? nM - first : GM;
      pm = first + (L % width) % gsz;
      pn = (L % width) / gsz;
    } else {
      pm = L / nN;
      pn = L % nN;
    }
    m0 = p.m_lo + pm * BMC;
    n0 = pn * BN;
#pragma unroll
    for (int h = 0; h < 2; ++h) {
#pragma unroll
      for (int i = 0; i < DA; ++i) {
        const int r = (i * 8 + wave) * 8 + (lane >> 3);
        const int c = (lane & 7) ^ ((r >> 1) & 7);
        int m = m0 + (r / (RA / 2)) * (BMC / 2) + h * (MF0 * FR) + r % (RA / 2);
        m = m < p.M ? m : p.M - 1;
        srcA[h][i] = Ag + (long)(m / p.rpb) * p.a_batch + (long)(m % p.rpb) * p.a_row + c * 8;
      }
#pragma unroll
      for (int i = 0; i < DB; ++i) {
        const int r = (i * 8 + wave) * 8 + (lane >> 3);
        const int c = (lane & 7) ^ ((r >> 1) & 7);
        int n = n0 + (r / (RB / 4)) * (BN / 4) + h * (RB / 4) + r % (RB / 4);
        n = n < p.N ? n : p.N - 1;
        srcB[h][i] = Wg + (long)n * p.ldw + c * 8;
      }
    }
  };
  const unsigned lds_base = (unsigned)(size_t)smem;
  auto dma16 = [&](const T* src, unsigned lds_off) {
    unsigned keep;
    const unsigned dst = __builtin_amdgcn_readfirstlane(lds_base + lds_off);
    asm volatile("s_mov_b32 %0, m0\n\ts_mov_b32 m0, %2\n\ts_nop 0\n\tglobal_load_lds_dwordx4 %1, off\n\ts_mov_b32 m0, %0"
                 : "=&s"(keep) : "v"(src), "s"(dst) : "memory");
  };
  auto koffA = [&](int kt) -> long { return (long)kt * 64; };
  auto koffB = [&](int kt) -> long { return (long)kt * 64; };
  auto stageA = [&](int h, int buf, int kt) {
    const long ko = koffA(kt);
#pragma unroll
    for (int i = 0; i < DA; ++i) dma16(srcA[h][i] + ko, buf * BUF + (h ? OFF_A1 : OFF_A0) + (i * 8 + wave) * 1024);
  };
  auto stageB = [&](int h, int buf, int kt) {
// ... 222 lines not shown
    quadrant(1, 1);
    quadrant(1, 0);
    AFX_BAR();
  };
  auto issue_prologue_r3 = [&] {
    stageB3(0, 0, 0);
    stageB3(1, 0, 0);
    stageA3(0, 0, 0);
    stageA3(1, 0, 0);
    if (nk > 1) {
      stageB3(0, 1, 1);
      stageB3(1, 1, 1);
      stageA3(0, FSZ3, 1);
      stageA3(1, FSZ3, 1);
    }
  };
  auto issue_prologue2 = [&] {
    stageR(0, 0, 0);
    stageR(1, 0, 0);
    stageF(0, 0, 0);
    stageF(1, 0, 0);
    if (nk > 1) {
      stageR(0, 1, 1);
      stageR(1, 1, 1);
      stageF(0, 1, 1);
    }
  };
  int v = blockIdx.x;
  setup(v);
  if constexpr (PH == 3) issue_prologue_r3(); else if constexpr (PH != 0) issue_prologue2(); else issue_prologue();
  bool first = true;
  for (;;) {
    if constexpr (PH == 3) {
      if (first && nk > 1) wait_vmcnt<2 * DA + 2 * DB>();
      else wait_vmcnt<0>();
    } else if constexpr (PH != 0) {
      constexpr int NF1 = WIDE ? DB : DA, NRRF = 2 * (WIDE ? DA : DB) + (WIDE ? DB : DA);
      if (first && nk > 1) wait_vmcnt<NF1 + NRRF>();
      else if (first) wait_vmcnt<NF1>();
      else wait_vmcnt<0>();
    } else {
      if (first && nk > 1) wait_vmcnt<6>();
      else wait_vmcnt<0>();
    }
    first = false;
    AFX_BAR();
    if (wr == 1) AFX_BAR();
#pragma unroll
    for (int i = 0; i < MF0 + MF1; ++i)
#pragma unroll
      for (int j = 0; j < 2 * NTH; ++j) acc[i][j] = 0.f;
    __builtin_amdgcn_s_waitcnt(0x0F70);
    for (int t = 0; t < nk; t += 2) {
      if constexpr (PH == 3) {
        const int f0 = (t % 3) * FSZ3, f1 = ((t + 1) % 3) * FSZ3, f2 = ((t + 2) % 3) * FSZ3;
        ktile_r3(std::integral_constant<int, 0>{}, t, f0, f2);
        if (t + 1 < nk) ktile_r3(std::integral_constant<int, 1>{}, t + 1, f1, f0);
      } else if constexpr (PH == 1) {
        ktile2(std::integral_constant<int, 0>{}, t);
        if (t + 1 < nk) ktile2(std::integral_constant<int, 1>{}, t + 1);
      } else {
        ktile(std::integral_constant<int, 0>{}, t);
        if (t + 1 < nk) ktile(std::integral_constant<int, 1>{}, t + 1);
      }
    }
    if (wr == 0) AFX_BAR();
    const int m0c = m0, n0c = n0;
    const int vn = v + gridDim.x;
    if (vn < nwg) {
      setup(vn);
      if constexpr (PH == 3) issue_prologue_r3(); else if constexpr (PH != 0) issue_prologue2(); else issue_prologue();
    }
    if (AFX_DBG(p, 64)) {
#pragma unroll
      for (int i = 0; i < MF0 + MF1; ++i)
#pragma unroll
        for (int j = 0; j < 2 * NTH; ++j)
#pragma unroll
          for (int r = 0; r < 4; ++r) asm volatile("" :: "v"(acc[i][j][r]));
    } else {
      gemm_epilogue<HT, BMC, BN, 2, 4, ROWLN, true, S3, ROWTAB>(p, acc, smem + BUF + (WIDE ? OFF_B1 : OFF_A1), m0c, n0c, g);
    }
    ts_on = false;
    if (vn >= nwg) break;
    v = vn;
  }
  if constexpr (TS) {
    __syncthreads();
    if (blockIdx.x == 0 && p.out_h)
      for (int i = tid; i < 8 * 16 * 16; i += 512) ((unsigned long long*)p.out_h)[i] = ts_lds[i];
  }
#undef AFX_BAR
}

template <class HT, int BM, int BN, bool ROWLN, int MF = BM / 32, int PH = 1, bool TS = false, bool S3 = false, bool ROWTAB = false>
static hipError_t launch_gemm8_t(const GemmArgs& p, int groups, hipStream_t s) {
  constexpr int lds = 2 * (BM + BN) * 128 + (TS ? 16384 : 0) + (PH == 3 ? BM * 128 : 0);
  static_assert(lds <= 160 * 1024, "two K-tile buffers must fit the 160 KB LDS");
  static LdsLimit lim;
  if (hipError_t e = lim.ensure((const void*)gemm8_kernel<HT, BM, BN, ROWLN, MF, PH, TS, S3, ROWTAB>, lds); e != hipSuccess) return e;
  static int n_cu_of[kMaxDevices] = {0};
  int dev = 0;
  if (hipGetDevice(&dev) != hipSuccess || dev < 0 || dev >= kMaxDevices) return hipErrorInvalidDevice;
  if (!n_cu_of[dev]) {
    int cus = 0;
    if (hipDeviceGetAttribute(&cus, hipDeviceAttributeMultiprocessorCount, dev) != hipSuccess) return hipErrorUnknown;
    cus &= ~7;
    n_cu_of[dev] = cus < 8 ? 8 : cus;
  }
  const int n_cu = n_cu_of[dev];
  const int tiles = ((p.N + BN - 1) / BN) * ((p.M - p.m_lo + MF * 32 - 1) / (MF * 32));
  dim3 grid(tiles < n_cu ? tiles : n_cu, 1, groups);
  hipLaunchKernelGGL((gemm8_kernel<HT, BM, BN, ROWLN, MF, PH, TS, S3, ROWTAB>), grid, dim3(512), lds, s, p);
  return hipGetLastError();
}

#ifdef AFX_ATTR
template <class HT>
__global__ __launch_bounds__(256) void gemm4_kernel(GemmArgs p) {
  typedef typename HT::T T;
  typedef typename HT::V8 V8;
  constexpr int STAGE = 512 * 128;
  constexpr int NP = 16;
  extern __shared__ __attribute__((aligned(16))) char smem[];
  const int tid = threadIdx.x, lane = tid & 63;
  const int wave = __builtin_amdgcn_readfirstlane(tid >> 6);
  const int wr = wave >> 1, wc = wave & 1;
  const int g = blockIdx.z;
  const T* Ag = (const T*)p.A + (long)g * p.g_a;
  const T* Wg = (const T*)p.W + (long)g * p.g_w;
  const int nN = (p.N + 255) / 256, nM = (p.M + 255) / 256;
  const int nwg = nM * nN;
  const int nk = p.K >> 6;
  const T* src[NP];
  int m0 = 0, n0 = 0;
  auto setup = [&](int v) {
    int pm, pn;
    int L = v;
    if (p.map_mode >= 1) {
      const int q = nwg >> 3, r = nwg & 7, xcd = L & 7;
      L = (xcd < r ? xcd * (q + 1) : r * (q + 1) + (xcd - r) * q) + (L >> 3);
    }
    if (p.map_mode == 2) {
      constexpr int GM = 8;
      const int width = GM * nN, grp = L / width, first = grp * GM;
      const int gsz = nM - first < GM ? nM - first : GM;
      pm = first + (L % width) % gsz;
      pn = (L % width) / gsz;
    } else {
      pm = L / nN;
      pn = L % nN;
    }
    m0 = pm * 256;
    n0 = pn * 256;
#pragma unroll
    for (int i = 0; i < NP; ++i) {
      const int row = (i * 4 + wave) * 8 + (lane >> 3);
      const int c = (lane & 7) ^ ((row >> 1) & 7);
      if (i < NP / 2) {
        int m = m0 + row;
        m = m < p.M ? m : p.M - 1;
        src[i] = Ag + (long)(m / p.rpb) * p.a_batch + (long)(m % p.rpb) * p.a_row + c * 8;
      } else {
        int n = n0 + row - 256;
        n = n < p.N ? n : p.N - 1;
        src[i] = Wg + (long)n * p.ldw + c * 8;
      }
    }
  };
  const unsigned lds_base = (unsigned)(size_t)smem;
  auto dma16 = [&](const T* s_, unsigned lds_off) {
    unsigned keep;
    const unsigned dst = __builtin_amdgcn_readfirstlane(lds_base + lds_off);
    asm volatile("s_mov_b32 %0, m0\n\ts_mov_b32 m0, %2\n\ts_nop 0\n\tglobal_load_lds_dwordx4 %1, off\n\ts_mov_b32 m0, %0"
                 : "=&s"(keep) : "v"(s_), "s"(dst) : "memory");
  };
  auto issue_tile = [&](int buf, int kt) {
    const long ko = (long)kt * 64;
#pragma unroll
    for (int i = 0; i < NP; ++i) dma16(src[i] + ko, buf * STAGE + (i * 4 + wave) * 1024);
  };
  const int frow = lane & 15, fsw = (frow >> 1) & 7, kq = lane >> 4;
  const char* aR = smem + (wr * 128 + frow) * 128;
  const char* bR = smem + (256 + wc * 128 + frow) * 128;
  auto read_frags = [&](int buf, int ks, V8 (&af)[8], V8 (&wf)[8]) {
    const int slot = ((ks * 4 + kq) ^ fsw) * 16;
#pragma unroll
    for (int j = 0; j < 8; ++j) wf[j] = *(const V8*)(bR + buf * STAGE + j * (16 * 128) + slot);
#pragma unroll
    for (int i = 0; i < 8; ++i) af[i] = *(const V8*)(aR + buf * STAGE + i * (16 * 128) + slot);
  };
  f32x4 acc[8][8];
  auto read_one = [&](int buf, int ks, int q, V8 (&af)[8], V8 (&wf)[8]) {
    const int slot = ((ks * 4 + kq) ^ fsw) * 16;
    if (q < 8) wf[q] = *(const V8*)(bR + buf * STAGE + q * (16 * 128) + slot);
    else af[q - 8] = *(const V8*)(aR + buf * STAGE + (q - 8) * (16 * 128) + slot);
// ... 614 lines not shown
      const int mf = gemm8_fit_mf(p, obj);
      const double whole = (double)gemm8_tiles(p, mf) * (mf + 5);
      const double split = (double)t1 * 13 + (double)((p.M - m1 + 127) / 128) * nN128 * kUnit128;
      if (g_fit == 1 && whole <= split) m1 = 0;
    } else {
      long fitted = 0;
      gemm8_fit_mf(p, OBJ_MAKESPAN, &fitted);
      const long split = ((t1 + 255) / 256) * 13 + 10;
      if (g_fit == 1 && fitted <= split) m1 = 0;
    }
  }
  if (m1 > 0) {
    pl.tile = 7;
    pl.rows = 256;
    pl.tiles = (long)(m1 / 256) * ((p.N + 255) / 256);
    pl.split_rows = m1;
    pl.rem_tile = 0;
    pl.rem_tiles = (long)((p.M - m1 + 127) / 128) * nN128;
    return pl;
  }
  if (tile == 7) {
    const int mf = gemm8_fit_mf(p, obj);
    if (mf < 8) tile = 70 + mf;
    pl.rows = mf * 32;
    pl.tiles = gemm8_tiles(p, mf);
  } else if (tile == 8) {
    const int mf = gemm8_fit_rowln(p, obj);
    if (mf < 4) tile = 80 + mf;
    pl.rows = mf * 32;
    pl.tiles = (p.M - p.m_lo + mf * 32 - 1) / (mf * 32);
    const long t128 = (p.M + 127) / 128, frac = t128 % 256;
    if (mf == 4 && g_fit == 1 && g_conv_split && t128 > 256 && frac != 0 && p.K >= 1536 && p.m_lo == 0) {
      const long head = (t128 / 256) * 256, rem64 = (p.M - head * 128 + 63) / 64;
      const bool take = dispatch_cu(obj, CU_SPLITS) ? head * 10 + rem64 * 8 < t128 * 10 : frac <= 96;
      if (take) {
        pl.tiles = head;
        pl.split_rows = (int)(head * 128);
        pl.rem_tile = 82;
        pl.rem_tiles = rem64;
      }
    }
  } else {
    const int bm = tile == 2 ? 256 : 128, bn = tile == 2 ? 256 : (tile == 3 ? 512 : (tile == 1 || tile == 92 ? 64 : 128));
    pl.rows = bm;
    pl.tiles = (long)((p.M + bm - 1) / bm) * ((p.N + bn - 1) / bn) * groups;
  }
  pl.tile = tile;
  return pl;
}

template <class HT>
static hipError_t dispatch(const GemmArgs& p, int tile, int groups, hipStream_t s) {
  const bool lean = (p.act == ACT_NONE || p.act == ACT_GELU) && (p.N & 7) == 0 && !(AFX_DBG(p, 16));
  switch (tile) {
    case 1: return lean ? launch_gemm_t<HT, 128, 64, 2, 2, false, true>(p, groups, s) : launch_gemm_t<HT, 128, 64, 2, 2>(p, groups, s);
    case 2: return launch_gemm_t<HT, 256, 256, 2, 4>(p, groups, s);
    case 3: return launch_gemm_t<HT, 128, 512, 2, 4, true>(p, groups, s);
#ifdef AFX_ATTR
    case 90: return launch_gemm_deep_t<HT, 128, 128, 2, 2, 4>(p, groups, s);
    case 91: return launch_gemm_deep_t<HT, 128, 128, 2, 4, 4>(p, groups, s);
    case 93: return launch_gemm_deep_t<HT, 128, 128, 2, 2, 3>(p, groups, s);
#endif
    case 92: return launch_gemm_deep_t<HT, 128, 64, 2, 2, 3>(p, groups, s);
#ifdef AFX_ATTR
    case 4: return launch_gemm4_t<HT>(p, groups, s);
    case 5: return launch_gemm5_t<HT>(p, groups, s);
#endif
    case 7:
      if (g_ph4 == 0) return launch_gemm8_t<HT, 256, 256, false, 8, 3>(p, groups, s);
#ifdef AFX_ATTR
      if (p.dbg_nodma & 8192) return launch_gemm8_t<HT, 256, 256, false, 8, 1, true>(p, groups, s);
#endif
      return g_ph4 == 1 ? launch_gemm8_t<HT, 256, 256, false, 8, 0>(p, groups, s) : launch_gemm8_t<HT, 256, 256, false>(p, groups, s);
    case 75: return g_ph4 == 0 ? launch_gemm8_t<HT, 256, 256, false, 5, 3>(p, groups, s) : launch_gemm8_t<HT, 256, 256, false, 5>(p, groups, s);
    case 76: return g_ph4 == 0 ? launch_gemm8_t<HT, 256, 256, false, 6, 3>(p, groups, s) : launch_gemm8_t<HT, 256, 256, false, 6>(p, groups, s);
    case 77: return g_ph4 == 0 ? launch_gemm8_t<HT, 256, 256, false, 7, 3>(p, groups, s) : launch_gemm8_t<HT, 256, 256, false, 7>(p, groups, s);
    case 8: return g_ph4 ? launch_gemm8_t<HT, 128, 512, true, 4, 0>(p, groups, s) : launch_gemm8_t<HT, 128, 512, true>(p, groups, s);
    case 82: return launch_gemm8_t<HT, 128, 512, true, 2>(p, groups, s);
    case 83: return launch_gemm8_t<HT, 128, 512, true, 3>(p, groups, s);
    default: return lean ? launch_gemm_t<HT, 128, 128, 2, 2, false, true>(p, groups, s) : launch_gemm_t<HT, 128, 128, 2, 2>(p, groups, s);
  }
}

static hipError_t dispatch_s3(const GemmArgs& p, int tile, int groups, hipStream_t s) {
  typedef FP16 HT;
  const bool lean = (p.act == ACT_NONE || p.act == ACT_GELU) && (p.N & 7) == 0;
  switch (tile) {
    case 1: return lean ? launch_gemm_t<HT, 128, 64, 2, 2, false, true, true>(p, groups, s) : launch_gemm_t<HT, 128, 64, 2, 2, false, false, true>(p, groups, s);
    case 92: return launch_gemm_deep_t<HT, 128, 64, 2, 2, 3, true>(p, groups, s);
    case 7: return launch_gemm8_t<HT, 256, 256, false, 8, 3, false, true>(p, groups, s);
    case 75: return launch_gemm8_t<HT, 256, 256, false, 5, 3, false, true>(p, groups, s);
    case 76: return launch_gemm8_t<HT, 256, 256, false, 6, 3, false, true>(p, groups, s);
    case 77: return launch_gemm8_t<HT, 256, 256, false, 7, 3, false, true>(p, groups, s);
    case 3:
    case 8: return launch_gemm8_t<HT, 128, 512, true, 4, 1, false, true>(p, groups, s);
    case 82: return launch_gemm8_t<HT, 128, 512, true, 2, 1, false, true>(p, groups, s);
    case 83: return launch_gemm8_t<HT, 128, 512, true, 3, 1, false, true>(p, groups, s);
    default: return lean ? launch_gemm_t<HT, 128, 128, 2, 2, false, true, true>(p, groups, s) : launch_gemm_t<HT, 128, 128, 2, 2, false, false, true>(p, groups, s);
  }
}
#define AFX_DISPATCH_GEMM(p, tile) ((p).k1 ? dispatch_s3(p, tile, groups, s) : (dtype == DT_BF16 ? dispatch<BF16>(p, tile, groups, s) : dispatch<FP16>(p, tile, groups, s)))

const char* launch_gemm(const GemmArgs& p_in, int dtype, int groups, hipStream_t s) {
  if (dtype == DT_FP32) return launch_gemm_f32(p_in, groups, s);
  if ((dtype == DT_FP16X3) != (p_in.k1 != 0)) return "gemm: the split-precision fields (k1, planes, column scales) go with DT_FP16X3 and only with it";
  if (const char* e = check_gemm(p_in, groups)) return e;
  GemmArgs p = p_in;
  p.map_mode = g_map_override >= 0 ? g_map_override : 2;
  const GemmPlan pl = gemm_plan(p, groups, dispatch_objective(p.objective));
  p.a_nt = g_ant_override >= 0 ? g_ant_override : (pl.tile == 3 ? 1 : 0);
  p.dbg_nodma = g_nodma;
  if (pl.split_rows > 0 && pl.tile == 7) {
    const int m1 = pl.split_rows;
    const size_t hs = 2;
    GemmArgs a = p, b = p;
    a.M = m1; a.rpb = m1; a.o_batch_rows = m1; a.oh_batch_rows = m1;
    b.M = p.M - m1; b.rpb = b.M; b.o_batch_rows = b.M; b.oh_batch_rows = b.M;
    b.A = (const char*)p.A + (size_t)m1 * p.a_row * hs;
    if (p.resid) b.resid = p.resid + (size_t)m1 * p.ldr;
    if (p.out_f) b.out_f = p.out_f + (size_t)m1 * p.ldo_f;
    if (p.out_h) b.out_h = (char*)p.out_h + (size_t)m1 * p.ldo_h * (p.k1 ? 4 : hs);
    hipError_t err = AFX_DISPATCH_GEMM(a, 7);
    if (err == hipSuccess) err = AFX_DISPATCH_GEMM(b, pl.rem_tile);
    return err == hipSuccess ? nullptr : hipGetErrorString(err);
  }
  if (pl.split_rows > 0) {
    GemmArgs a = p, b = p;
    a.M = pl.split_rows;
    b.m_lo = a.M;
    hipError_t err = AFX_DISPATCH_GEMM(a, pl.tile);
    if (err == hipSuccess) err = AFX_DISPATCH_GEMM(b, pl.rem_tile);
    return err == hipSuccess ? nullptr : hipGetErrorString(err);
  }
  const hipError_t err = AFX_DISPATCH_GEMM(p, pl.tile);
  return err == hipSuccess ? nullptr : hipGetErrorString(err);
}

const char* launch_gemm_rows(const GemmArgs& p_in, int dtype, hipStream_t s) {
  if (dtype == DT_FP32) return "gemm_rows: half- or split-precision operands only";
  if ((dtype == DT_FP16X3) != (p_in.k1 != 0)) return "gemm: the split-precision fields (k1, planes, column scales) go with DT_FP16X3 and only with it";
  if (const char* e = check_gemm(p_in, 1)) return e;
  if (!p_in.oh_rows || !p_in.out_h || p_in.out_f || p_in.resid || p_in.ln_gamma || !plain_k(p_in) || (p_in.N & 7) ||
      (p_in.act != ACT_NONE && p_in.act != ACT_GELU) || p_in.m_lo)
    return "gemm_rows: operand-type output with a row table, plain K, N % 8 == 0, no LayerNorm / fp32 output / residual";
  GemmArgs p = p_in;
  p.map_mode = g_map_override >= 0 ? g_map_override : 2;
  p.a_nt = g_ant_override >= 0 ? g_ant_override : 0;
  p.dbg_nodma = g_nodma;
  const bool wide = gemm_tile_of(p, 1) == 7;
  hipError_t err;
  if (p.k1)
    err = wide ? launch_gemm8_t<FP16, 256, 256, false, 8, 3, false, true, true>(p, 1, s)
               : launch_gemm_t<FP16, 128, 128, 2, 2, false, true, true, true>(p, 1, s);
  else if (dtype == DT_BF16)
    err = wide ? launch_gemm8_t<BF16, 256, 256, false, 8, 3, false, false, true>(p, 1, s)
               : launch_gemm_t<BF16, 128, 128, 2, 2, false, true, false, true>(p, 1, s);
  else
    err = wide ? launch_gemm8_t<FP16, 256, 256, false, 8, 3, false, false, true>(p, 1, s)
               : launch_gemm_t<FP16, 128, 128, 2, 2, false, true, false, true>(p, 1, s);
  return err == hipSuccess ? nullptr : hipGetErrorString(err);
}

}
```

### real-time-deepfake-speech-detection_amd/csrc/afx_kernels.h

```cpp
#pragma once
#include <hip/hip_runtime.h>
#include <stdint.h>

namespace afx {

enum DType { DT_BF16 = 0, DT_FP16 = 1, DT_FP32 = 2, DT_FP16X3 = 3 };
inline size_t dtype_size(int dt) { return dt == DT_FP32 || dt == DT_FP16X3 ? 4 : 2; }
constexpr float kS3ScaleBounded = 16.f;
constexpr float kS3ScaleFree = 1.f;
__host__ __device__ inline long s3_pair_index(long k) { return ((k >> 5) << 6) + (k & 31); }

struct GemmArgs {
  const void* A;
  const void* W;
  int M, N, K;
  int k_algo;
  int rpb;
  long a_batch, a_row;
  int kchunk;
  long kchunk_stride;
  long ldw;
  long g_a, g_w;
  int g_n;
  const float* bias;
  int act;
  float alpha;
  const float* resid;
  long ldr;
  float* out_f;
  long ldo_f;
  void* out_h;
  long ldo_h;
  int o_batch_rows, o_row_off;
  union {
    struct {
      int oh_batch_rows, oh_row_off;
    };
    const int* oh_rows;
  };
  int map_mode;
  const float* ln_gamma;
  const float* ln_beta;
  float ln_eps;
  int a_nt;
  int no_deep;
  int m_lo;
  int k1;
  int objective;
  const float* pre_scale;
  float a_inv;
  int oh_pairs;
  float oh_scale;
  int dbg_nodma;
};
const char* launch_gemm(const GemmArgs& p, int dtype, int groups, hipStream_t s);
const char* launch_gemm_rows(const GemmArgs& p, int dtype, hipStream_t s);
const char* launch_gemm_f32(const GemmArgs& p, int groups, hipStream_t s);
bool gemm_is_narrow(int N);
int gemm_tile_of(const GemmArgs& p, int groups);
enum { OBJ_MAKESPAN = 0, OBJ_CU_TIME = 1 };
enum { CU_GEMM8_HEIGHT = 1, CU_CHAIN_WAVES = 2, CU_ROWLN_HEIGHT = 4, CU_SPLITS = 8 };
void dispatch_force_objective(int obj);
void dispatch_set_cu_mask(int mask);
int dispatch_objective(int of_launch);
bool dispatch_cu(int obj, int bit);
struct GemmPlan {
  int family;
  int tile;
  int rows;
  long tiles;
  int split_rows;
  int rem_tile;
  long rem_tiles;
};
GemmPlan gemm_plan(const GemmArgs& p, int groups, int objective);
void gemm_set_s3_small(int v);
void gemm_set_map_mode(int m);
void gemm_set_small_deep(int v);
void gemm_set_tile(int t);
void gemm_set_a_nt(int v);
void gemm_set_conv_split(int v);
void gemm_set_ph4(int v);
void gemm_set_fit(int v);
void gemm_set_split(int v);
void mhsa_set_zsplit(int v);
void mhsa_set_waves(int v);
void mhsa_set_force_long(int v);
void conf_attn_mfma_set_waves(int v);
void conf_attn_mfma_set_force_long(int v);
void conf_attn_set_block(int v);
void gemm_set_deep(int v);
bool gemm_set_nodma(int v);

const char* launch_conv0(const float* wave, int B, int L, int T0, const float* w ,
                         const float* bias, const float* gamma, const float* beta, int pre_emph,
                         float pre_coef, void* out_h, int dtype, hipStream_t s, const void* wpack = nullptr, float pair_scale = 0.f);
size_t conv0_pack_bytes();
const char* launch_conv0_pack(const float* w , const float* bias, void* pack, hipStream_t s);
const char* launch_conv0_groupnorm(const float* wave, int B, int L, int T0, const float* w, const float* gamma,
                                   const float* beta, float eps, float* stats, void* out_h, int dtype, hipStream_t s);
size_t conv0_groupnorm_stats_floats(int B, int T0);
const char* launch_tile_crop(const float* x, const long long* offs, const long long* starts, int B, int duration,
                             float* out, hipStream_t s);
void conv0_set_mfma(int v);
const char* launch_pre_emphasis(const float* x, int B, int L, float coef, float* y, hipStream_t s);
struct RowNormArgs {
  const float* x;
  long ldx;
  int rows, C;
  const float* gamma;
  const float* beta;
  float eps;
  int act;
  float* out_f;
  long ldo_f;
  void* out_h;
  long ldo_h;
  int rpb, o_batch_rows, o_row_off;
  int* nonfinite;
  const int* nf_lens;
  int nf_rpb;
  int oh_pairs;
  float oh_scale;
};
const char* launch_rownorm(const RowNormArgs& a, int dtype, hipStream_t s);
const char* launch_zero_pad_rows(void* buf_h, int B, int T, int C, int pad_front, int pad_back, int dtype,
                                 hipStream_t s, const int* lens = nullptr);
const char* launch_pack_linear(const float* w, int N, int K, int Kpad, void* out_h, int dtype, hipStream_t s);
const char* launch_pack_conv(const float* w, int N, int Cin, int k, void* out_h, int dtype, hipStream_t s);
const char* launch_pack_posconv(const float* v, const float* g, int C, int cpg, int k, float* norm_tmp ,
                                void* out_h, int dtype, hipStream_t s);
const char* launch_split_weight_rows(void* w_f32_inplace, int N, int K, float* row_scale, hipStream_t s);
const char* launch_split_pairs(const float* x, long n, void* pairs, float scale, hipStream_t s);

struct PosConvArgs {
  const void* xpad;
  long xpad_batch;
  const void* W;
  const float* bias;
  float* x;
  int B, T, slab_rows;
};
const char* launch_posconv(const PosConvArgs& p, int dtype, hipStream_t s);

const char* launch_mhsa(const void* qkv, void* out, int B, int T, int H, int dtype, hipStream_t s, const int* lens = nullptr);
void mhsa_set_vtr(int v);

const char* launch_mhsa_split(const float* qkv, float* out, int B, int T, int H, hipStream_t s, const int* lens = nullptr,
                              bool out_pairs = false, float out_scale = 1.f);
struct MhsaRingForm {
  int form;
  int q_tile;
  const int* cnt;
  const int* tab;
};
const char* launch_mhsa_ring(const void* ring, void* out, int S, int H, const MhsaRingForm& f, int dtype, hipStream_t s);
const char* launch_mhsa_ring_split(const float* ring, float* out, int S, int H, const MhsaRingForm& f, hipStream_t s,
                                   bool out_pairs = false, float out_scale = 1.f);
// ... 43 lines not shown
```

Measured before the change: 13900.

## Fuse LayerNorm into residual GEMM epilogue via per-panel completion counters

Adds a GEMM variant whose epilogue, once all column tiles of a 160-row panel finish (tracked by atomic counters), normalises those rows and writes the half-precision LayerNorm output. The trunk uses it for the attention-output and FFN-down residual products, so the separate ln2 and next-layer ln1 rownorm launches are skipped. This removes extra kernel launches and a re-read of the fp32 residual stream. In exchange it adds a memset of counters per forward, cross-block synchronisation through atomics, and tail work done by whichever block finishes a panel last. It is gated on a dispatch objective bit, so it may not run by default.

After: 13760. 1.0% lower.

```diff
diff --git a/include/afx.h b/include/afx.h
--- a/include/afx.h
+++ b/include/afx.h
@@ -97,6 +97,7 @@
 int afx_engine_get(afx_handle h, const char* key, int* value);
 int afx_gemm_plan(int M, int N, int K, int rpb, int kchunk, int groups, int flags, int objective, int* out);
 int afx_conf_chain_waves(int M, int objective);
+int afx_gemm_ln_tail(int M, int N, int K, int flags, int objective);
 int afx_debug_set(const char* key, int value);
 
 int afx_k_gemm(int dtype, const void* A, long lda, const void* W, long ldw, int M, int N, int K, const float* bias,
@@ -104,6 +105,10 @@
                void* stream);
 int afx_k_conv_gemm(int dtype, const void* in_h, const void* Wp, int B, int Tin, int Tout, int Cin, int k, int s,
                     int N, const float* bias, float* out_f, void* stream);
+int afx_k_gemm_ln_counters(int M);
+int afx_k_gemm_ln(int dtype, const void* A, long lda, const void* W, long ldw, int M, int N, int K, const float* bias,
+                  int act, float alpha, const float* resid, long ldr, float* out_f, long ldo_f, void* out_h, long ldo_h,
+                  const float* gamma, const float* beta, float eps, void* ln_out, long ld_ln, void* cnt, void* stream);
 int afx_k_conv_ln_act(int dtype, const void* in_h, const void* Wp, int B, int Tin, int Tout, int Cin, int k, int s,
                       const float* bias, const float* gamma, const float* beta, float eps, int act, float* out_f,
                       void* out_h, void* stream);
diff --git a/real-time-deepfake-speech-detection_amd/afx/_lib.py b/real-time-deepfake-speech-detection_amd/afx/_lib.py
--- a/real-time-deepfake-speech-detection_amd/afx/_lib.py
+++ b/real-time-deepfake-speech-detection_amd/afx/_lib.py
@@ -67,6 +67,7 @@
     "afx_engine_get": (_I, [_P, C.c_char_p, C.POINTER(C.c_int)]),
     "afx_gemm_plan": (_I, [_I, _I, _I, _I, _I, _I, _I, _I, C.POINTER(C.c_int)]),
     "afx_conf_chain_waves": (_I, [_I, _I]),
+    "afx_gemm_ln_tail": (_I, [_I, _I, _I, _I, _I]),
     "afx_kv_create": (_I, [_P, _I, C.POINTER(_P)]),
     "afx_kv_destroy": (None, [_P]),
     "afx_kv_state_bytes": (_Z, [_P]),
@@ -89,6 +90,8 @@
     "afx_profile_class_name": (C.c_char_p, [_I]),
     "afx_debug_set": (_I, [C.c_char_p, _I]),
     "afx_k_gemm": (_I, [_I, _P, _L, _P, _L, _I, _I, _I, _P, _I, _F, _P, _L, _P, _L, _P, _L, _P]),
+    "afx_k_gemm_ln_counters": (_I, [_I]),
+    "afx_k_gemm_ln": (_I, [_I, _P, _L, _P, _L, _I, _I, _I, _P, _I, _F, _P, _L, _P, _L, _P, _L, _P, _P, _F, _P, _L, _P, _P]),
     "afx_k_conv_gemm": (_I, [_I, _P, _P, _I, _I, _I, _I, _I, _I, _I, _P, _P, _P]),
     "afx_k_conv_ln_act": (_I, [_I, _P, _P, _I, _I, _I, _I, _I, _I, _P, _P, _P, _F, _I, _P, _P, _P]),
     "afx_k_pack_linear": (_I, [_I, _P, _I, _I, _I, _P, _P]),
diff --git a/real-time-deepfake-speech-detection_amd/afx/kernels.py b/real-time-deepfake-speech-detection_amd/afx/kernels.py
--- a/real-time-deepfake-speech-detection_amd/afx/kernels.py
+++ b/real-time-deepfake-speech-detection_amd/afx/kernels.py
@@ -24,6 +24,20 @@
                            alpha, ptr(resid), N if resid is None else resid.stride(0), ptr(of), N if of is None else of.stride(0),
                            ptr(oh), N if oh is None else oh.stride(0)))
     return of, oh
+
+
+def gemm_ln(dtype, A, W, gamma, beta, eps=1e-5, bias=None, act=None, alpha=1.0, resid=None, out_f=True, out_h=False, ln_out=True):
+    M, K = A.shape
+    N = W.shape[0]
+    of = _out(out_f, (M, N), torch.float32, A.device)
+    oh = _out(out_h, (M, N), torch_dtype(dtype), A.device)
+    ln = _out(ln_out, (M, N), torch_dtype(dtype), A.device)
+    cnt = torch.empty(lib().afx_k_gemm_ln_counters(M), dtype=torch.int32, device=A.device)
+    check(call_on(A, lib().afx_k_gemm_ln, DTYPES[dtype], ptr(A), A.stride(0), ptr(W), W.stride(0), M, N, K, ptr(bias), ACTS[act],
+                  alpha, ptr(resid), N if resid is None else resid.stride(0), ptr(of), N if of is None else of.stride(0),
+                  ptr(oh), N if oh is None else oh.stride(0), ptr(gamma), ptr(beta), eps, ptr(ln), N if ln is None else ln.stride(0),
+                  ptr(cnt)))
+    return of, oh, ln
 
 
 def pack_linear(dtype, w, kpad=None):
diff --git a/real-time-deepfake-speech-detection_amd/csrc/afx_engine.hip b/real-time-deepfake-speech-detection_amd/csrc/afx_engine.hip
--- a/real-time-deepfake-speech-detection_amd/csrc/afx_engine.hip
+++ b/real-time-deepfake-speech-detection_amd/csrc/afx_engine.hip
@@ -684,6 +684,8 @@
   void* s3planes = nullptr;
   size_t s3bytes = 0;
   float* gn_stats = nullptr;
+  unsigned* ln_cnt = nullptr;
+  size_t ln_cnt_bytes = 0;
   int* lens = nullptr;
   float *bucket_f = nullptr, *bucket_logits = nullptr;
   float *ll32 = nullptr, *xc = nullptr, *qkv32 = nullptr, *glu32 = nullptr;
@@ -751,6 +753,13 @@
     w->s3bytes = big + 4096;
     w->s3planes = c.take(w->s3bytes);
   }
+  w->ln_cnt = nullptr;
+  w->ln_cnt_bytes = 0;
+  if ((L > 0 || T5 > 0) && (e->dt == AFX_DT_FP16 || e->dt == AFX_DT_BF16) && e->cfg.n_layers > 0) {
+    const size_t words = (size_t)2 * e->cfg.n_layers * gemm_ln_tail_panels(B * (T > 0 ? T : 1));
+    w->ln_cnt_bytes = (words * 4 + 15) & ~(size_t)15;
+    w->ln_cnt = (unsigned*)c.take(w->ln_cnt_bytes);
+  }
   return c.off + 256;
 }
 
@@ -877,6 +886,7 @@
   }
   const char* gemm(const GemmArgs& g_in, int dt, int groups, bool rows = false);
   const char* rownorm(const RowNormArgs& a_in, const LnW& ln, int dt);
+  const char* gemm_ln(const GemmArgs& g_in, const LnW& ln, void* out, long ldo, unsigned* cnt, int dt);
 };
 const char* Call::gemm(const GemmArgs& g_in, int dt, int groups, bool rows) {
   GemmArgs g = g_in;
@@ -930,6 +940,13 @@
   if (rows && (dt == DT_FP32 || groups != 1)) return "gemm with a row table: half- or split-precision operands, one group";
   return timed(dt == DT_FP32 ? PC_GEMM_F32 : cls_of(gemm_tile_of(g, groups)), fl,
                [&] { return rows ? launch_gemm_rows(g, dt, s) : launch_gemm(g, dt, groups, s); });
+}
+const char* Call::gemm_ln(const GemmArgs& g_in, const LnW& ln, void* out, long ldo, unsigned* cnt, int dt) {
+  GemmArgs g = g_in;
+  g.no_deep = e->gemm_small_deep ? 0 : 1;
+  g.objective = objective;
+  const GemmLnTail t{ln.g, ln.b, kLnEps, out, ldo, cnt};
+  return timed(PC_GEMM8_256, 2.0 * g.M * g.N * (g.k_algo ? g.k_algo : g.K), [&] { return launch_gemm_ln(g, t, dt, s); });
 }
 const char* Call::rownorm(const RowNormArgs& a_in, const LnW& ln, int dt) {
   RowNormArgs a = a_in;
@@ -1127,16 +1144,36 @@
     KOK(posconv_product(cx, w.xpad, Tt + kPosK, B, Tt, w.x, dt));
   }
   if (tap(cx, "pos", w.x, (size_t)M * kD, false)) return 1;
-  auto resid_product = [&](const void* A, long lda, const void* W, int K, const float* bias) -> const char* {
+  auto resid_args = [&](const void* A, long lda, const void* W, int K, const float* bias) {
     GemmArgs o = plain_gemm(A, lda, W, K, M, kD, K);
     o.bias = bias; o.resid = w.x; o.ldr = kD; o.out_f = w.x; o.ldo_f = kD;
+    return o;
+  };
+  bool tail_o = false, tail_2 = false;
+  const int ln_panels = gemm_ln_tail_panels(M);
+  if ((dt == DT_FP16 || dt == DT_BF16) && w.ln_cnt && dispatch_cu(dispatch_objective(cx.objective), CU_LN_TAIL)) {
+    auto takes = [&](int K) {
+      GemmArgs o = resid_args(nullptr, K, nullptr, K, nullptr);
+      o.no_deep = e->gemm_small_deep ? 0 : 1;
+      return gemm_ln_tail_refusal(o, 1, dispatch_objective(cx.objective)) == nullptr;
+    };
+    tail_o = takes(kD);
+    tail_2 = e->cfg.n_layers > 1 && takes(kF);
+    if (tail_o || tail_2) HIP_OK(hipMemsetAsync(w.ln_cnt, 0, w.ln_cnt_bytes, s));
+  }
+  auto resid_product = [&](const void* A, long lda, const void* W, int K, const float* bias, const LnW* ln, int ordinal) -> const char* {
+    const GemmArgs o = resid_args(A, lda, W, K, bias);
+    if (ln) return cx.gemm_ln(o, *ln, w.hbuf, kD, w.ln_cnt + (size_t)ordinal * ln_panels, dt);
     return cx.gemm(o, dt, 1);
   };
+  bool have_ln1 = false;
   for (int l = 0; l < e->cfg.n_layers; ++l) {
     const TrunkLayer& L = e->layers[l];
-    RowNormArgs n1 = plain_norm(w.x, kD, M, kD);
-    n1.out_h = w.hbuf; n1.ldo_h = kD;
-    KOK(cx.rownorm(n1, L.ln1, dt));
+    if (!have_ln1) {
+      RowNormArgs n1 = plain_norm(w.x, kD, M, kD);
+      n1.out_h = w.hbuf; n1.ldo_h = kD;
+      KOK(cx.rownorm(n1, L.ln1, dt));
+    }
     auto lp = [l](const char* leaf) { return "l" + std::to_string(l) + "." + leaf; };
     TAP(lp("ln1"), w.hbuf, (size_t)M * kD, true, kD);
     GemmArgs q = plain_gemm(w.hbuf, kD, L.wqkv, kD, M, 3 * kD, kD);
@@ -1154,18 +1191,21 @@
       return launch_mhsa(w.qkv, w.att, B, Tt, kH, dt, s, w.lens);
     }));
     TAP(lp("att"), w.att, (size_t)M * kD, true, kD);
-    KOK(resid_product(w.att, kD, L.wo, kD, L.bo));
+    KOK(resid_product(w.att, kD, L.wo, kD, L.bo, tail_o ? &L.ln2 : nullptr, 2 * l));
     TAP(lp("mid"), w.x, (size_t)M * kD, false, kD);
-    RowNormArgs n2 = plain_norm(w.x, kD, M, kD);
-    n2.out_h = w.hbuf; n2.ldo_h = kD;
-    KOK(cx.rownorm(n2, L.ln2, dt));
+    if (!tail_o) {
+      RowNormArgs n2 = plain_norm(w.x, kD, M, kD);
+      n2.out_h = w.hbuf; n2.ldo_h = kD;
+      KOK(cx.rownorm(n2, L.ln2, dt));
+    }
     TAP(lp("ln2"), w.hbuf, (size_t)M * kD, true, kD);
     GemmArgs f1 = plain_gemm(w.hbuf, kD, L.w1, kD, M, kF, kD);
     f1.bias = L.b1; f1.act = ACT_GELU;
     f1.out_h = w.ff; f1.ldo_h = kF;
     KOK(cx.gemm(f1, dt, 1));
     TAP(lp("ff"), w.ff, (size_t)M * kF, true, kF);
-    KOK(resid_product(w.ff, kF, L.w2, kF, L.b2));
+    have_ln1 = tail_2 && l + 1 < e->cfg.n_layers;
+    KOK(resid_product(w.ff, kF, L.w2, kF, L.b2, have_ln1 ? &e->layers[l + 1].ln1 : nullptr, 2 * l + 1));
     if (e->taps_on) {
       const std::string nm = "layer" + std::to_string(l);
       if (tap(cx, nm.c_str(), w.x, (size_t)M * kD, false)) return 1;
@@ -2361,6 +2401,19 @@
   }
   KRET(launch_gemm(g, dtype, 1, (hipStream_t)stream));
 }
+extern "C" int afx_k_gemm_ln_counters(int M) { return M > 0 ? (gemm_ln_tail_panels(M) + 3) & ~3 : 0; }
+extern "C" int afx_k_gemm_ln(int dtype, const void* A, long lda, const void* W, long ldw, int M, int N, int K,
+                             const float* bias, int act, float alpha, const float* resid, long ldr, float* out_f,
+                             long ldo_f, void* out_h, long ldo_h, const float* gamma, const float* beta, float eps,
+                             void* ln_out, long ld_ln, void* cnt, void* stream) {
+  if (!cnt || M <= 0) return fail("afx_k_gemm_ln: the panel counters (afx_k_gemm_ln_counters(M) words) are required");
+  GemmArgs g = plain_gemm(A, lda, W, ldw, M, N, K);
+  g.bias = bias; g.act = act; g.alpha = alpha; g.resid = resid; g.ldr = ldr;
+  g.out_f = out_f; g.ldo_f = ldo_f; g.out_h = out_h; g.ldo_h = ldo_h;
+  HIP_OK(hipMemsetAsync(cnt, 0, (size_t)afx_k_gemm_ln_counters(M) * 4, (hipStream_t)stream));
+  const GemmLnTail t{gamma, beta, eps, ln_out, ld_ln, (unsigned*)cnt};
+  KRET(launch_gemm_ln(g, t, dtype, (hipStream_t)stream));
+}
 extern "C" int afx_k_conv_gemm(int dtype, const void* in_h, const void* Wp, int B, int Tin, int Tout, int Cin, int k,
                                int s_, int N, const float* bias, float* out_f, void* stream) {
   GemmArgs g = plain_gemm(in_h, 0, Wp, (long)k * Cin, B * Tout, N, k * Cin);
@@ -2551,6 +2604,20 @@
   out[4] = pl.split_rows; out[5] = pl.rem_tile; out[6] = (int)pl.rem_tiles; out[7] = obj;
   return 0;
 }
+extern "C" int afx_gemm_ln_tail(int M, int N, int K, int flags, int objective) {
+  if (M <= 0 || N <= 0 || K <= 0) { (void)fail("afx_gemm_ln_tail: bad arguments"); return -1; }
+  static float dummy;
+  GemmArgs g = plain_gemm(nullptr, K, nullptr, K, M, N, K);
+  g.out_f = &dummy; g.resid = &dummy;
+  if (flags & 2) { g.k1 = K; g.K = 2 * K; g.kchunk = 2 * g.kchunk; }
+  if (flags & 4) g.act = ACT_SWISH;
+  if (flags & 8) g.no_deep = 1;
+  if (flags & 16) g.rpb = (M + 1) / 2 > 0 ? (M + 1) / 2 : 1;
+  const int obj = objective < 0 ? dispatch_objective(OBJ_MAKESPAN) : (objective ? OBJ_CU_TIME : OBJ_MAKESPAN);
+  if (!dispatch_cu(obj, CU_LN_TAIL)) { (void)fail("afx_gemm_ln_tail: the LayerNorm tail is a CU-time decision (objective, dispatch_cu_mask bit 16)"); return 0; }
+  if (const char* m = gemm_ln_tail_refusal(g, 1, obj)) { (void)fail("%s", m); return 0; }
+  return 1;
+}
 extern "C" int afx_conf_chain_waves(int M, int objective) {
   return conf_chain_waves_of(M, objective < 0 ? dispatch_objective(OBJ_MAKESPAN) : (objective ? OBJ_CU_TIME : OBJ_MAKESPAN));
 }
diff --git a/real-time-deepfake-speech-detection_amd/csrc/afx_frontend.hip b/real-time-deepfake-speech-detection_amd/csrc/afx_frontend.hip
--- a/real-time-deepfake-speech-detection_amd/csrc/afx_frontend.hip
+++ b/real-time-deepfake-speech-detection_amd/csrc/afx_frontend.hip
@@ -2,6 +2,7 @@
 
 #include "afx_common.h"
 #include "afx_kernels.h"
+#include "afx_rownorm.h"
 
 namespace afx {
 
@@ -577,99 +578,11 @@
 
 template <class HT, int RPW>
 __global__ __launch_bounds__(256) void rownorm_kernel(RowNormArgs a) {
-  typedef typename HT::T T;
-  typedef typename HT::V4 V4;
   const int lane = threadIdx.x & 63;
   const long r0 = ((long)blockIdx.x * 4 + (threadIdx.x >> 6)) * RPW;
   if (r0 >= a.rows) return;
-  f32x4 v[RPW][4];
-  bool live[RPW];
-#pragma unroll
-  for (int u = 0; u < RPW; ++u) {
-    live[u] = r0 + u < a.rows;
-    const float* x = a.x + (live[u] ? r0 + u : r0) * a.ldx;
-#pragma unroll
-    for (int it = 0; it < 4; ++it) {
-      const int c = (it * 64 + lane) * 4;
-      v[u][it] = f32x4{0.f, 0.f, 0.f, 0.f};
-      if (c < a.C) v[u][it] = *(const f32x4*)(x + c);
-    }
-  }
   f32x4 gm[4], bt[4];
-#pragma unroll
-  for (int it = 0; it < 4; ++it) {
-    const int c = (it * 64 + lane) * 4;
-    gm[it] = bt[it] = f32x4{0.f, 0.f, 0.f, 0.f};
-    if (c < a.C) {
-      gm[it] = *(const f32x4*)(a.gamma + c);
-      bt[it] = *(const f32x4*)(a.beta + c);
-    }
-  }
-  const float inv = 1.0f / (float)a.C;
-#pragma unroll
-  for (int u = 0; u < RPW; ++u) {
-    if (!live[u]) continue;
-    const long r = r0 + u;
-    float sum = 0.f;
-#pragma unroll
-    for (int it = 0; it < 4; ++it) sum += (v[u][it][0] + v[u][it][1]) + (v[u][it][2] + v[u][it][3]);
-    const float mean = wave_sum(sum) * inv;
-    float sq = 0.f;
-#pragma unroll
-    for (int it = 0; it < 4; ++it) {
-      const int c = (it * 64 + lane) * 4;
-      if (c < a.C) {
-#pragma unroll
-        for (int i = 0; i < 4; ++i) {
-          v[u][it][i] -= mean;
-          sq = fmaf(v[u][it][i], v[u][it][i], sq);
-        }
-      }
-    }
-    const float var = wave_sum(sq) * inv;
-    const float rstd = 1.0f / sqrtf(var + a.eps);
-    if (a.nonfinite && lane == 0 && !(fabsf(mean) <= 3.0e38f && var <= 3.0e38f) &&
-        (!a.nf_lens || (int)(r % a.nf_rpb) < a.nf_lens[r / a.nf_rpb]))
-      atomicAdd(a.nonfinite, 1);
-    const long orow = (r / a.rpb) * a.o_batch_rows + (r % a.rpb) + a.o_row_off;
-    auto emit = [&](auto with_act) {
-#pragma unroll
-      for (int it = 0; it < 4; ++it) {
-        const int c = (it * 64 + lane) * 4;
-        if (c < a.C) {
-          const f32x4 g = gm[it], b = bt[it];
-          f32x4 y;
-#pragma unroll
-          for (int i = 0; i < 4; ++i) {
-            y[i] = fmaf(v[u][it][i] * rstd, g[i], b[i]);
-            if (decltype(with_act)::value) y[i] = apply_act(y[i], a.act);
-          }
-          if (a.out_f) *(f32x4*)(a.out_f + orow * a.ldo_f + c) = y;
-          if (a.out_h) {
-            if (std::is_same<T, float>::value && a.oh_pairs) {
-              f16x4 hi, lo;
-#pragma unroll
-              for (int i = 0; i < 4; ++i) {
-                const float sv = y[i] * a.oh_scale;
-                hi[i] = (_Float16)sv;
-                lo[i] = (_Float16)(sv - (float)hi[i]);
-              }
-              _Float16* hp = (_Float16*)a.out_h + orow * (2 * a.ldo_h) + s3_pair_index(c);
-              *(f16x4*)hp = hi;
-              *(f16x4*)(hp + 32) = lo;
-            } else {
-              V4 h;
-#pragma unroll
-              for (int i = 0; i < 4; ++i) h[i] = (T)y[i];
-              *(V4*)((T*)a.out_h + orow * a.ldo_h + c) = h;
-            }
-          }
-        }
-      }
-    };
-    if (a.act == ACT_NONE) emit(std::false_type{});
-    else emit(std::true_type{});
-  }
+  rownorm_rows<HT, RPW>(a, r0, lane, gm, bt);
 }
 
 const char* launch_rownorm(const RowNormArgs& a, int dtype, hipStream_t s) {
diff --git a/real-time-deepfake-speech-detection_amd/csrc/afx_gemm.hip b/real-time-deepfake-speech-detection_amd/csrc/afx_gemm.hip
--- a/real-time-deepfake-speech-detection_amd/csrc/afx_gemm.hip
+++ b/real-time-deepfake-speech-detection_amd/csrc/afx_gemm.hip
@@ -1,5 +1,6 @@
 #include "afx_common.h"
 #include "afx_kernels.h"
+#include "afx_rownorm.h"
 
 #include <type_traits>
 
@@ -7,6 +8,10 @@
 #define AFX_DBG(p, bit) ((p).dbg_nodma & (bit))
 #else
 #define AFX_DBG(p, bit) 0
+#endif
+
+#ifndef AFX_LNT_RPW
+#define AFX_LNT_RPW 4
 #endif
 
 namespace afx {
@@ -536,9 +541,11 @@
 }
 
 
-template <class HT, int BM, int BN, bool ROWLN, int MF = BM / 32, int PH = 1, bool TS = false, bool S3 = false, bool ROWTAB = false>
-__global__ __launch_bounds__(512) void gemm8_kernel(GemmArgs p) {
+template <class HT, int BM, int BN, bool ROWLN, int MF = BM / 32, int PH = 1, bool TS = false, bool S3 = false, bool ROWTAB = false,
+          bool LNT = false>
+__global__ __launch_bounds__(512) void gemm8_kernel(std::conditional_t<LNT, GemmArgsLnt, GemmArgs> p) {
   static_assert(!ROWTAB || !ROWLN, "per-batch output rows: wide-store epilogue only");
+  static_assert(!LNT || (PH == 3 && BM == 256 && BN == 256 && !ROWLN && !S3 && !ROWTAB && !TS), "LayerNorm tail: the 256-wide ring form");
   typedef typename HT::T T;
   typedef typename HT::V8 V8;
   constexpr bool WIDE = BN > BM;
@@ -927,6 +934,41 @@
       gemm_epilogue<HT, BMC, BN, 2, 4, ROWLN, true, S3, ROWTAB>(p, acc, smem + BUF + (WIDE ? OFF_B1 : OFF_A1), m0c, n0c, g);
     }
     ts_on = false;
+    if constexpr (LNT) {
+      constexpr int RPW = AFX_LNT_RPW;
+      unsigned* last_flag = (unsigned*)(smem + 2 * RSZ3 + 2 * FSZ3);
+      wait_vmcnt<0>();
+      __syncthreads();
+      if (tid == 0) {
+        __builtin_amdgcn_fence(__ATOMIC_RELEASE, "agent");
+        asm volatile("s_waitcnt vmcnt(0)" ::: "memory");
+        const unsigned ticket = __hip_atomic_fetch_add(p.lnt.cnt + m0c / BMC, 1u, __ATOMIC_RELAXED, __HIP_MEMORY_SCOPE_AGENT);
+        const bool last = ticket == (unsigned)(nN - 1);
+        if (last) {
+          __builtin_amdgcn_fence(__ATOMIC_ACQUIRE, "agent");
+          asm volatile("s_waitcnt vmcnt(0)" ::: "memory");
+        }
+        *last_flag = last ? 1u : 0u;
+      }
+      __syncthreads();
+      if (*last_flag) {
+        int lane_t = lane;
+        asm volatile("" : "+v"(lane_t));
+        RowNormArgs a;
+        a.x = p.out_f; a.ldx = p.ldo_f;
+        a.rows = m0c + BMC < p.M ? m0c + BMC : p.M;
+        a.C = p.N;
+        a.gamma = p.lnt.gamma; a.beta = p.lnt.beta; a.eps = p.lnt.eps; a.act = ACT_NONE;
+        a.out_f = nullptr; a.ldo_f = 0;
+        a.out_h = p.lnt.out; a.ldo_h = p.lnt.ldo;
+        a.rpb = p.M; a.o_batch_rows = p.M; a.o_row_off = 0;
+        a.nonfinite = nullptr; a.nf_lens = nullptr; a.nf_rpb = 1;
+        a.oh_pairs = 0; a.oh_scale = 1.f;
+        f32x4 gm[4], bt[4];
+        rownorm_affine(a, lane_t, gm, bt);
+        for (long r0 = m0c + wave * RPW; r0 < a.rows; r0 += 8 * RPW) rownorm_rows<HT, RPW, true>(a, r0, lane_t, gm, bt);
+      }
+    }
     if (vn >= nwg) break;
     v = vn;
   }
@@ -937,13 +979,7 @@
   }
 #undef AFX_BAR
 }
-
-template <class HT, int BM, int BN, bool ROWLN, int MF = BM / 32, int PH = 1, bool TS = false, bool S3 = false, bool ROWTAB = false>
-static hipError_t launch_gemm8_t(const GemmArgs& p, int groups, hipStream_t s) {
-  constexpr int lds = 2 * (BM + BN) * 128 + (TS ? 16384 : 0) + (PH == 3 ? BM * 128 : 0);
-  static_assert(lds <= 160 * 1024, "two K-tile buffers must fit the 160 KB LDS");
-  static LdsLimit lim;
-  if (hipError_t e = lim.ensure((const void*)gemm8_kernel<HT, BM, BN, ROWLN, MF, PH, TS, S3, ROWTAB>, lds); e != hipSuccess) return e;
+static hipError_t gemm8_grid(long tiles, int* grid) {
   static int n_cu_of[kMaxDevices] = {0};
   int dev = 0;
   if (hipGetDevice(&dev) != hipSuccess || dev < 0 || dev >= kMaxDevices) return hipErrorInvalidDevice;
@@ -954,9 +990,19 @@
     n_cu_of[dev] = cus < 8 ? 8 : cus;
   }
   const int n_cu = n_cu_of[dev];
-  const int tiles = ((p.N + BN - 1) / BN) * ((p.M - p.m_lo + MF * 32 - 1) / (MF * 32));
-  dim3 grid(tiles < n_cu ? tiles : n_cu, 1, groups);
-  hipLaunchKernelGGL((gemm8_kernel<HT, BM, BN, ROWLN, MF, PH, TS, S3, ROWTAB>), grid, dim3(512), lds, s, p);
+  *grid = tiles < n_cu ? (int)tiles : n_cu;
+  return hipSuccess;
+}
+template <class HT, int BM, int BN, bool ROWLN, int MF = BM / 32, int PH = 1, bool TS = false, bool S3 = false, bool ROWTAB = false,
+          bool LNT = false>
+static hipError_t launch_gemm8_t(const std::conditional_t<LNT, GemmArgsLnt, GemmArgs>& p, int groups, hipStream_t s) {
+  constexpr int lds = 2 * (BM + BN) * 128 + (TS ? 16384 : 0) + (PH == 3 ? BM * 128 : 0);
+  static_assert(lds <= 160 * 1024, "two K-tile buffers must fit the 160 KB LDS");
+  static LdsLimit lim;
+  if (hipError_t e = lim.ensure((const void*)gemm8_kernel<HT, BM, BN, ROWLN, MF, PH, TS, S3, ROWTAB, LNT>, lds); e != hipSuccess) return e;
+  int g = 0;
+  if (hipError_t e = gemm8_grid((long)((p.N + BN - 1) / BN) * ((p.M - p.m_lo + MF * 32 - 1) / (MF * 32)), &g); e != hipSuccess) return e;
+  hipLaunchKernelGGL((gemm8_kernel<HT, BM, BN, ROWLN, MF, PH, TS, S3, ROWTAB, LNT>), dim3(g, 1, groups), dim3(512), lds, s, p);
   return hipGetLastError();
 }
 
@@ -1737,6 +1783,29 @@
   }
 }
 
+template <class HT>
+static hipError_t dispatch_lnt(const GemmArgsLnt& p, int tile, hipStream_t s) {
+  switch (tile) {
+    case 7: return launch_gemm8_t<HT, 256, 256, false, 8, 3, false, false, false, true>(p, 1, s);
+    case 75: return launch_gemm8_t<HT, 256, 256, false, 5, 3, false, false, false, true>(p, 1, s);
+    case 76: return launch_gemm8_t<HT, 256, 256, false, 6, 3, false, false, false, true>(p, 1, s);
+    case 77: return launch_gemm8_t<HT, 256, 256, false, 7, 3, false, false, false, true>(p, 1, s);
+    default: return hipErrorInvalidValue;
+  }
+}
+const char* gemm_ln_tail_refusal(const GemmArgs& p, int groups, int obj) {
+  if (groups != 1 || p.rpb < p.M) return "gemm: LayerNorm tail: one group and the plain row mapping only (rows-per-batch >= M)";
+  if (p.N != 512 && p.N != 768 && p.N != 1024) return "gemm: LayerNorm tail: N must be 512, 768 or 1024 (whole 256-wide tiles of a row one wave normalises)";
+  if (!p.out_f) return "gemm: LayerNorm tail: the rows are normalised from the fp32 output (out_f)";
+  if (p.k1) return "gemm: LayerNorm tail: not in split precision";
+  if (p.ln_gamma || !plain_k(p) || p.m_lo) return "gemm: LayerNorm tail: a plain product (no LayerNorm epilogue, no chunked K, all rows)";
+  if (g_ph4 != 0) return "gemm: LayerNorm tail: the ring form of the 256-wide kernel only (gemm_ph4 = 0)";
+  const GemmPlan pl = gemm_plan(p, groups, obj);
+  if (pl.family != 7 || pl.split_rows > 0 || !(pl.tile == 7 || (pl.tile >= 75 && pl.tile <= 77)))
+    return "gemm: LayerNorm tail: needs a single-kernel plan of the 8-phase 256-wide family (no round split, lean epilogue)";
+  return nullptr;
+}
+
 static hipError_t dispatch_s3(const GemmArgs& p, int tile, int groups, hipStream_t s) {
   typedef FP16 HT;
   const bool lean = (p.act == ACT_NONE || p.act == ACT_GELU) && (p.N & 7) == 0;
@@ -1788,6 +1857,28 @@
     return err == hipSuccess ? nullptr : hipGetErrorString(err);
   }
   const hipError_t err = AFX_DISPATCH_GEMM(p, pl.tile);
+  return err == hipSuccess ? nullptr : hipGetErrorString(err);
+}
+
+const char* launch_gemm_ln(const GemmArgs& p_in, const GemmLnTail& t, int dtype, hipStream_t s) {
+  if (dtype != DT_BF16 && dtype != DT_FP16) return "gemm: LayerNorm tail: half-precision operands only";
+  if (const char* e = check_gemm(p_in, 1)) return e;
+  const int obj = dispatch_objective(p_in.objective);
+  if (const char* e = gemm_ln_tail_refusal(p_in, 1, obj)) return e;
+  if (!t.gamma || !t.beta || !t.cnt || !t.out || ((size_t)t.gamma & 15) || ((size_t)t.beta & 15) || ((size_t)t.cnt & 3))
+    return "gemm: LayerNorm tail: gamma, beta (16-byte aligned), the output and the panel counters are required";
+  if (((size_t)t.out & 7) || (t.ldo & 3) || t.ldo < p_in.N || ((size_t)p_in.out_f & 15) || (p_in.ldo_f & 3))
+    return "gemm: LayerNorm tail: output rows must start on 8-byte boundaries (ldo % 4 == 0, >= N)";
+  if (t.out == p_in.A || t.out == p_in.W || t.out == (void*)p_in.out_f || t.out == p_in.out_h)
+    return "gemm: LayerNorm tail: the normalised rows need a buffer of their own";
+  GemmArgsLnt p;
+  static_cast<GemmArgs&>(p) = p_in;
+  p.lnt = t;
+  p.map_mode = g_map_override >= 0 ? g_map_override : 2;
+  const GemmPlan pl = gemm_plan(p, 1, obj);
+  p.a_nt = g_ant_override >= 0 ? g_ant_override : 0;
+  p.dbg_nodma = g_nodma;
+  const hipError_t err = dtype == DT_BF16 ? dispatch_lnt<BF16>(p, pl.tile, s) : dispatch_lnt<FP16>(p, pl.tile, s);
   return err == hipSuccess ? nullptr : hipGetErrorString(err);
 }
 
diff --git a/real-time-deepfake-speech-detection_amd/csrc/afx_kernels.h b/real-time-deepfake-speech-detection_amd/csrc/afx_kernels.h
--- a/real-time-deepfake-speech-detection_amd/csrc/afx_kernels.h
+++ b/real-time-deepfake-speech-detection_amd/csrc/afx_kernels.h
@@ -54,12 +54,24 @@
   int dbg_nodma;
 };
 const char* launch_gemm(const GemmArgs& p, int dtype, int groups, hipStream_t s);
+struct GemmLnTail {
+  const float* gamma;
+  const float* beta;
+  float eps;
+  void* out;
+  long ldo;
+  unsigned* cnt;
+};
+struct GemmArgsLnt : GemmArgs {
+  GemmLnTail lnt;
+};
+const char* launch_gemm_ln(const GemmArgs& p, const GemmLnTail& t, int dtype, hipStream_t s);
 const char* launch_gemm_rows(const GemmArgs& p, int dtype, hipStream_t s);
 const char* launch_gemm_f32(const GemmArgs& p, int groups, hipStream_t s);
 bool gemm_is_narrow(int N);
 int gemm_tile_of(const GemmArgs& p, int groups);
 enum { OBJ_MAKESPAN = 0, OBJ_CU_TIME = 1 };
-enum { CU_GEMM8_HEIGHT = 1, CU_CHAIN_WAVES = 2, CU_ROWLN_HEIGHT = 4, CU_SPLITS = 8 };
+enum { CU_GEMM8_HEIGHT = 1, CU_CHAIN_WAVES = 2, CU_ROWLN_HEIGHT = 4, CU_SPLITS = 8, CU_LN_TAIL = 16 };
 void dispatch_force_objective(int obj);
 void dispatch_set_cu_mask(int mask);
 int dispatch_objective(int of_launch);
@@ -74,6 +86,8 @@
   long rem_tiles;
 };
 GemmPlan gemm_plan(const GemmArgs& p, int groups, int objective);
+const char* gemm_ln_tail_refusal(const GemmArgs& p, int groups, int objective);
+inline int gemm_ln_tail_panels(int M) { return (M + 159) / 160; }
 void gemm_set_s3_small(int v);
 void gemm_set_map_mode(int m);
 void gemm_set_small_deep(int v);
diff --git a/real-time-deepfake-speech-detection_amd/csrc/afx_rownorm.h b/real-time-deepfake-speech-detection_amd/csrc/afx_rownorm.h
--- /dev/null
+++ b/real-time-deepfake-speech-detection_amd/csrc/afx_rownorm.h
@@ -0,0 +1,106 @@
+#pragma once
+#include "afx_common.h"
+#include "afx_kernels.h"
+
+#include <type_traits>
+
+namespace afx {
+
+__device__ __forceinline__ void rownorm_affine(const RowNormArgs& a, int lane, f32x4 (&gm)[4], f32x4 (&bt)[4]) {
+#pragma unroll
+  for (int it = 0; it < 4; ++it) {
+    const int c = (it * 64 + lane) * 4;
+    gm[it] = bt[it] = f32x4{0.f, 0.f, 0.f, 0.f};
+    if (c < a.C) {
+      gm[it] = *(const f32x4*)(a.gamma + c);
+      bt[it] = *(const f32x4*)(a.beta + c);
+    }
+  }
+}
+
+template <class HT, int RPW, bool HAVE_AFFINE = false>
+__device__ __forceinline__ void rownorm_rows(const RowNormArgs& a, long r0, int lane, f32x4 (&gm)[4], f32x4 (&bt)[4]) {
+  typedef typename HT::T T;
+  typedef typename HT::V4 V4;
+  f32x4 v[RPW][4];
+  bool live[RPW];
+#pragma unroll
+  for (int u = 0; u < RPW; ++u) {
+    live[u] = r0 + u < a.rows;
+    const float* x = a.x + (live[u] ? r0 + u : r0) * a.ldx;
+#pragma unroll
+    for (int it = 0; it < 4; ++it) {
+      const int c = (it * 64 + lane) * 4;
+      v[u][it] = f32x4{0.f, 0.f, 0.f, 0.f};
+      if (c < a.C) v[u][it] = *(const f32x4*)(x + c);
+    }
+  }
+  if constexpr (!HAVE_AFFINE) rownorm_affine(a, lane, gm, bt);
+  const float inv = 1.0f / (float)a.C;
+#pragma unroll
+  for (int u = 0; u < RPW; ++u) {
+    if (!live[u]) continue;
+    const long r = r0 + u;
+    float sum = 0.f;
+#pragma unroll
+    for (int it = 0; it < 4; ++it) sum += (v[u][it][0] + v[u][it][1]) + (v[u][it][2] + v[u][it][3]);
+    const float mean = wave_sum(sum) * inv;
+    float sq = 0.f;
+#pragma unroll
+    for (int it = 0; it < 4; ++it) {
+      const int c = (it * 64 + lane) * 4;
+      if (c < a.C) {
+#pragma unroll
+        for (int i = 0; i < 4; ++i) {
+          v[u][it][i] -= mean;
+          sq = fmaf(v[u][it][i], v[u][it][i], sq);
+        }
+      }
+    }
+    const float var = wave_sum(sq) * inv;
+    const float rstd = 1.0f / sqrtf(var + a.eps);
+    if (a.nonfinite && lane == 0 && !(fabsf(mean) <= 3.0e38f && var <= 3.0e38f) &&
+        (!a.nf_lens || (int)(r % a.nf_rpb) < a.nf_lens[r / a.nf_rpb]))
+      atomicAdd(a.nonfinite, 1);
+    const long orow = (r / a.rpb) * a.o_batch_rows + (r % a.rpb) + a.o_row_off;
+    auto emit = [&](auto with_act) {
+#pragma unroll
+      for (int it = 0; it < 4; ++it) {
+        const int c = (it * 64 + lane) * 4;
+        if (c < a.C) {
+          const f32x4 g = gm[it], b = bt[it];
+          f32x4 y;
+#pragma unroll
+          for (int i = 0; i < 4; ++i) {
+            y[i] = fmaf(v[u][it][i] * rstd, g[i], b[i]);
+            if (decltype(with_act)::value) y[i] = apply_act(y[i], a.act);
+          }
+          if (a.out_f) *(f32x4*)(a.out_f + orow * a.ldo_f + c) = y;
+          if (a.out_h) {
+            if (std::is_same<T, float>::value && a.oh_pairs) {
+              f16x4 hi, lo;
+#pragma unroll
+              for (int i = 0; i < 4; ++i) {
+                const float sv = y[i] * a.oh_scale;
+                hi[i] = (_Float16)sv;
+                lo[i] = (_Float16)(sv - (float)hi[i]);
+              }
+              _Float16* hp = (_Float16*)a.out_h + orow * (2 * a.ldo_h) + s3_pair_index(c);
+              *(f16x4*)hp = hi;
+              *(f16x4*)(hp + 32) = lo;
+            } else {
+              V4 h;
+#pragma unroll
+              for (int i = 0; i < 4; ++i) h[i] = (T)y[i];
+              *(V4*)((T*)a.out_h + orow * a.ldo_h + c) = h;
+            }
+          }
+        }
+      }
+    };
+    if (a.act == ACT_NONE) emit(std::false_type{});
+    else emit(std::true_type{});
+  }
+}
+
+}
```
